# dwave-examples/image-generation

Measured on AMD Instinct MI355X. Metric: DVAE+GRBM train-step images/s (MNIST) at 1/2/4/8 MI355X; loss parity vs CPU, higher is better.
Workload: dtype f32

## Files before the change

### image-generation_amd/csrc/common.h

```cpp
#pragma once
#include <hip/hip_runtime.h>
#include <atomic>
#include <stdint.h>
#include <stdio.h>
#include <stdarg.h>
#include "../../include/dvg.h"

namespace dvg {

void set_error(const char* fmt, ...);

#define DVG_CHECK_HIP(expr)                                                            \
  do {                                                                                 \
    hipError_t _e = (expr);                                                            \
    if (_e != hipSuccess) {                                                            \
      dvg::set_error("%s failed: %s (%s:%d)", #expr, hipGetErrorString(_e), __FILE__,  \
                     __LINE__);                                                        \
      return DVG_E_HIP;                                                                \
    }                                                                                  \
  } while (0)

#define DVG_REQUIRE(cond, ...)            \
  do {                                    \
    if (!(cond)) {                        \
      dvg::set_error(__VA_ARGS__);        \
      return DVG_E_INVALID;               \
    }                                     \
  } while (0)

#define DVG_TRY(expr)          \
  do {                         \
    int _rc = (expr);          \
    if (_rc != DVG_OK) return _rc; \
  } while (0)

enum KernelId : int {
  K_GIBBS = 0,
  K_GRBM_ENERGY,
  K_GRBM_SUFFSTATS,
  K_GUMBEL_FWD,
  K_GUMBEL_BWD,
  K_MMD_PREP,
  K_MMD_DISTSUM,
  K_MMD_MAIN,
  K_MMD_PM1,
  K_MMD_FINAL,
  K_IGEMM_128x64,
  K_IGEMM_64x64,
  K_IGEMM_128x32,
  K_IGEMM_32x64,
  K_IGEMM_128x128,
  K_WGRAD_2x2,
  K_WGRAD_2x1,
  K_WGRAD_1x2,
  K_WGRAD_1x1,
  K_WGRAD_FOLD,
  K_WGRAD_REDUCE,
  K_WEIGHT_PACK,
  K_BN_FINALIZE,
  K_ENC_CONV0_FWD,
  K_ENC_CONV0_WGRAD,
  K_ENC_BN_POOL_FWD,
  K_ENC_BN_POOL_BWD_REDUCE,
  K_ENC_BN_POOL_BWD_APPLY,
  K_ENC_PROJ_FWD,
  K_ENC_PROJ_BWD,
  K_DEC_BN_ACT_FWD,
  K_DEC_BN_ACT_BWD_REDUCE,
  K_DEC_BN_ACT_BWD_APPLY,
  K_DEC_CONV3_FWD,
  K_DEC_CONV3_BWD,
  K_DEC_FINAL_FWD,
  K_DEC_FINAL_BWD,
  K_MSE,
  K_ADAM,
  K_MISC,
  K_IGEMM_WSPACE,
  K_IGEMM_WINO,
  K_WGRAD_WINO,
  K_IGEMM_WINO4,
  K_WGRAD_WINO4,
  K_COUNT
};

enum Opt : int {
  OPT_IGEMM_DMA = 0, OPT_IGEMM_POSMAJOR, OPT_IGEMM_THR128, OPT_WGRAD_DMA, OPT_DEC_FOLD, OPT_DEC_D22, OPT_DEC_LC0, OPT_MMD_W128,
  OPT_MMD_D256, OPT_GIBBS_GENERIC, OPT_SIDE_STREAM, OPT_ENC_WINO, OPT_DEC_WINO, OPT_ENC_L0_FUSED, OPT_DEC_TAIL_FUSED,
  OPT_WINO_DYNAMIC, OPT_ENC_WINO4, OPT_ENC_WINO4_MASK, OPT_ENC_DGRAD_CUS, OPT_ENC_WGRAD_CUS, OPT_DEC_WINO4_MASK, OPT_WGRAD_REDUCE_TILED, OPT_ENC_BN_REDUCE_POOLED, OPT_COUNT
};
int64_t opt(Opt id);

bool side_enabled();
void side_stream_warm();
int* dyn_tile_counters();
hipStream_t side_stream(hipStream_t fallback);
int stream_order_after(hipStream_t waiter, hipStream_t producer);
int prep_arm(const void* ws, uint64_t sig, hipStream_t producer);
int prep_join(const void* ws, uint64_t sig, hipStream_t waiter, bool* armed, bool* matched);
int stream_mark(hipStream_t producer, hipEvent_t* mark);
int stream_wait_mark(hipStream_t waiter, hipEvent_t mark);

bool prof_on(int id);
void prof_begin(int id, hipStream_t s);
void prof_end(int id, hipStream_t s, double work, float share);

struct ProfScope {
  int id; hipStream_t s; bool on; double work; float share;
  ProfScope(int id_, hipStream_t s_, double work_ = 0.0, float share_ = 1.0f) : id(id_), s(s_), on(prof_on(id_)), work(work_), share(share_) {
    if (on) prof_begin(id, s);
  }
  ~ProfScope() { if (on) prof_end(id, s, work, share); }
};

#define DVG_LAUNCH(id, kernel, grid, block, shmem, stream, ...) \
  DVG_LAUNCH_WORK(id, 0.0, kernel, grid, block, shmem, stream, __VA_ARGS__)

#define DVG_LAUNCH_WORK(id, work, kernel, grid, block, shmem, stream, ...) \
  DVG_LAUNCH_WORK_SHARE(id, work, 1.0f, kernel, grid, block, shmem, stream, __VA_ARGS__)

#define DVG_LAUNCH_WORK_SHARE(id, work, share, kernel, grid, block, shmem, stream, ...) \
  do {                                                                                  \
    dvg::ProfScope _ps((id), (stream), (work), (share));                                \
    hipLaunchKernelGGL(kernel, grid, block, shmem, stream, __VA_ARGS__);                \
    hipError_t _le = hipGetLastError();                                                 \
    if (_le != hipSuccess) {                                                            \
      dvg::set_error("launch of %s failed: %s (%s:%d)", #kernel, hipGetErrorString(_le), \
                     __FILE__, __LINE__);                                               \
      return DVG_E_HIP;                                                                 \
    }                                                                                   \
  } while (0)

static inline int raise_dynamic_lds(std::atomic<uint64_t>& done, const void* kern, int bytes) {
  int dev = 0;
  DVG_CHECK_HIP(hipGetDevice(&dev));
  const uint64_t bit = 1ull << (dev & 63);
  if (!(done.load(std::memory_order_acquire) & bit)) {
    DVG_CHECK_HIP(hipFuncSetAttribute(kern, hipFuncAttributeMaxDynamicSharedMemorySize, bytes));
    done.fetch_or(bit, std::memory_order_release);
  }
  return DVG_OK;
}

static inline int64_t ceil_div(int64_t a, int64_t b) { return (a + b - 1) / b; }
static inline size_t align_up(size_t a, size_t b) { return (a + b - 1) / b * b; }

}
```

### image-generation_amd/csrc/mmd.hip

```cpp
#include <cstdlib>
#include <type_traits>

#include "common.h"

namespace dvg {

typedef float f32x16 __attribute__((ext_vector_type(16)));
typedef float f32x4 __attribute__((ext_vector_type(4)));
typedef int i32x4 __attribute__((ext_vector_type(4)));
typedef int i32x16 __attribute__((ext_vector_type(16)));

struct MmdArgs {
  const float* x; const float* y;
  int64_t nx, ny;
  int d;
  const float* sq;
  const float* coef;
  int n_kernels, squared, reduce_mean, biased;
  int pow2;
  double* loss_part;
  int vgx = 0, vgy = 0, vgz = 0;
  float* grad_part;
  int S;
  double* dist_part;
  const int8_t* zi8;
  const int* not_pm1;
  int pm1_ok;
  int gate_main;
  const uint16_t* zt;
  int64_t ztb_y;
  const uint4* tab;
};

constexpr int MMD_BI = 32;
constexpr int MMD_BJ = 128;
constexpr int MMD_PITCH = 33;

__device__ __forceinline__ int crow(int r, int hh) { return (r & 3) + 8 * (r >> 2) + 4 * hh; }

__device__ __forceinline__ f32x16 gram_tile(const float* __restrict__ src_i, int64_t cnt_i, int64_t base_i,
                                            const float* __restrict__ src_j, int64_t cnt_j, int64_t base_j, int d,
                                            float* Zs, float* Xs) {
  const int tid = threadIdx.x, lane = tid & 63, wave = tid >> 6;
  const int hh = lane >> 5, c = lane & 31;
  f32x16 acc = {0};
  const int nchunk = d / 32;
  f32x4 zreg[4], xreg;
  float zmask[4], xmask;
  auto load_chunk = [&](int ch) {
#pragma unroll
    for (int q = 0; q < 4; ++q) {
      const int idx = tid + 256 * q;
      const int row = idx >> 3, c4 = idx & 7;
      const int64_t gr = base_j + row;
      const bool okz = gr < cnt_j;
      zreg[q] = *reinterpret_cast<const f32x4*>(src_j + (okz ? gr * d + ch * 32 + c4 * 4 : 0));
      zmask[q] = okz ? 1.0f : 0.0f;
    }
    const int row = tid >> 3, c4 = tid & 7;
    const int64_t gr = base_i + row;
    const bool okx = gr < cnt_i;
    xreg = *reinterpret_cast<const f32x4*>(src_i + (okx ? gr * d + ch * 32 + c4 * 4 : 0));
    xmask = okx ? 1.0f : 0.0f;
  };
  load_chunk(0);
  for (int ch = 0; ch < nchunk; ++ch) {
    __syncthreads();
#pragma unroll
    for (int q = 0; q < 4; ++q) {
      const int idx = tid + 256 * q;
      const int row = idx >> 3, c4 = idx & 7;
      float* p = Zs + row * MMD_PITCH + c4 * 4;
      p[0] = zreg[q].x * zmask[q]; p[1] = zreg[q].y * zmask[q]; p[2] = zreg[q].z * zmask[q]; p[3] = zreg[q].w * zmask[q];
    }
    {
      const int row = tid >> 3, c4 = tid & 7;
      float* p = Xs + row * MMD_PITCH + c4 * 4;
      p[0] = xreg.x * xmask; p[1] = xreg.y * xmask; p[2] = xreg.z * xmask; p[3] = xreg.w * xmask;
    }
    __syncthreads();
    if (ch + 1 < nchunk) load_chunk(ch + 1);
    const float* za = Zs + (wave * 32 + c) * MMD_PITCH + hh;
    const float* xb = Xs + c * MMD_PITCH + hh;
#pragma unroll
    for (int s = 0; s < 16; ++s) acc = __builtin_amdgcn_mfma_f32_32x32x2f32(za[2 * s], xb[2 * s], acc, 0, 0, 0);
  }
  return acc;
}

constexpr int MMD_I8_PANEL = 512;

template <int ROWS>
struct I8Stage {
  i32x4 v[ROWS / 32][4];
  __device__ __forceinline__ void load(const int8_t* __restrict__ src, int d, int64_t base, int64_t cnt, int n16) {
    const int tr = threadIdx.x >> 3, tc = threadIdx.x & 7;
#pragma unroll
    for (int q = 0; q < 4; ++q) {
      if (q * 8 < n16) {
        const int c16 = q * 8 + tc < n16 ? q * 8 + tc : n16 - 1;
#pragma unroll
        for (int p = 0; p < ROWS / 32; ++p) {
          int64_t gr = base + tr + 32 * p;
          gr = gr < cnt ? gr : cnt - 1;
          v[p][q] = *reinterpret_cast<const i32x4*>(src + gr * d + c16 * 16);
        }
      }
    }
  }
  __device__ __forceinline__ void store(int8_t* dst, int pitch, int n16) const {
    const int tr = threadIdx.x >> 3, tc = threadIdx.x & 7;
#pragma unroll
    for (int q = 0; q < 4; ++q) {
      if (q * 8 < n16) {
        const int c16 = q * 8 + tc < n16 ? q * 8 + tc : n16 - 1;
#pragma unroll
        for (int p = 0; p < ROWS / 32; ++p)
          *reinterpret_cast<i32x4*>(dst + (tr + 32 * p) * pitch + c16 * 16) = v[p][q];
      }
    }
  }
};

__device__ __forceinline__ f32x16 gram_tile_i8(const int8_t* __restrict__ zi8, int64_t goff_i, int64_t cnt_i,
                                               int64_t base_i, int64_t goff_j, int64_t cnt_j, int64_t base_j, int d,
                                               int8_t* Zs8, int8_t* Xs8) {
  const int tid = threadIdx.x, lane = tid & 63, wave = tid >> 6;
  const int hh = lane >> 5, c = lane & 31;
  const int pw = d < MMD_I8_PANEL ? d : MMD_I8_PANEL;
  const int pitch = pw + 16;
  i32x16 acc = {0};
  for (int c0 = 0; c0 < d; c0 += MMD_I8_PANEL) {
    const int cw = d - c0 < MMD_I8_PANEL ? d - c0 : MMD_I8_PANEL;
    const int n16 = cw >> 4;
    I8Stage<MMD_BJ> zst;
    I8Stage<MMD_BI> xst;
    zst.load(zi8 + goff_j * d + c0, d, base_j, cnt_j, n16);
    xst.load(zi8 + goff_i * d + c0, d, base_i, cnt_i, n16);
    __syncthreads();
    zst.store(Zs8, pitch, n16);
    xst.store(Xs8, pitch, n16);
    __syncthreads();
    const int8_t* za = Zs8 + (wave * 32 + c) * pitch + hh * 16;
    const int8_t* xb = Xs8 + c * pitch + hh * 16;
    for (int s = 0; s < (cw >> 5); ++s)
      acc = __builtin_amdgcn_mfma_i32_32x32x32_i8(*reinterpret_cast<const i32x4*>(za + s * 32),
                                                  *reinterpret_cast<const i32x4*>(xb + s * 32), acc, 0, 0, 0);
  }
  f32x16 out;
#pragma unroll
  for (int r = 0; r < 16; ++r) out[r] = (float)acc[r];
  return out;
}

__device__ __forceinline__ void mmd_pair_terms(float D, const float (&ck)[8], int nk, bool pow2, float& ks, float& kp) {
  ks = 0.f; kp = 0.f;
  if (pow2) {
    float e = expf(ck[nk - 1] * D);
#pragma unroll
    for (int k = 7; k >= 0; --k) {
      if (k < nk) {
        ks += e;
        kp = fmaf(ck[k], e, kp);
        e *= e;
      }
    }
  } else {
#pragma unroll
    for (int k = 0; k < 8; ++k) {
      if (k < nk) {
        const float e = expf(ck[k] * D);
        ks += e;
        kp = fmaf(ck[k], e, kp);
      }
    }
  }
}

__device__ __forceinline__ double block_sum(double v, double* red) {
  const int tid = threadIdx.x;
  red[tid] = v;
  __syncthreads();
  for (int s = 128; s > 0; s >>= 1) {
    if (tid < s) red[tid] += red[tid + s];
    __syncthreads();
  }
  const double r = red[0];
  __syncthreads();
  return r;
}

__global__ __launch_bounds__(256) void mmd_prep_kernel(const float* __restrict__ x, int64_t nx,
                                                       const float* __restrict__ y, int64_t ny, int d,
                                                       float* __restrict__ sq, int8_t* __restrict__ zi8,
                                                       int* __restrict__ not_pm1) {
  const int64_t row = (int64_t)blockIdx.x * 4 + (threadIdx.x >> 6);
  const int lane = threadIdx.x & 63;
  if (row >= nx + ny) return;
  const float* p = row < nx ? x + row * d : y + (row - nx) * d;
  float acc = 0.f;
  bool bad = false;
  uint32_t* z4 = reinterpret_cast<uint32_t*>(zi8 + row * d);
  for (int k = lane; k < d / 4; k += 64) {
    const float4 v = *reinterpret_cast<const float4*>(p + 4 * k);
    acc = fmaf(v.x, v.x, acc); acc = fmaf(v.y, v.y, acc); acc = fmaf(v.z, v.z, acc); acc = fmaf(v.w, v.w, acc);
    bad |= !(v.x == 1.0f || v.x == -1.0f) | !(v.y == 1.0f || v.y == -1.0f) | !(v.z == 1.0f || v.z == -1.0f) | !(v.w == 1.0f || v.w == -1.0f);
    z4[k] = (v.x > 0.f ? 0x01u : 0xffu) | (v.y > 0.f ? 0x0100u : 0xff00u) | (v.z > 0.f ? 0x010000u : 0xff0000u) |
            (v.w > 0.f ? 0x01000000u : 0xff000000u);
  }
  if (__any(bad) && lane == 0) atomicOr(not_pm1, 1);
#pragma unroll
  for (int off = 32; off > 0; off >>= 1) acc += __shfl_down(acc, off, 64);
  if (lane == 0) sq[row] = acc;
}

template <int NS>
__device__ __forceinline__ void mmd_distsum_spin128(const MmdArgs& a, unsigned char* dsm) {
  double* red = reinterpret_cast<double*>(dsm);
  float* Dtab = reinterpret_cast<float*>(dsm + 2048);
  const int d = a.d, pw = d < MMD_I8_PANEL ? d : MMD_I8_PANEL, zp = pw + 16;
  int8_t* Zs8 = reinterpret_cast<int8_t*>(dsm + 2048 + ((d + 1) * 4 + 15) / 16 * 16);
  for (int h = threadIdx.x; h <= d; h += 256) {
    const float d2 = (float)(4 * h);
    Dtab[h] = a.squared ? d2 : sqrtf(d2);
  }
  const int64_t tx = (a.nx + MMD_BJ - 1) / MMD_BJ, ty = (a.ny + MMD_BJ - 1) / MMD_BJ, T = tx + ty;
  const int lane = threadIdx.x & 63, wave = threadIdx.x >> 6, hh = lane >> 5, c = lane & 31;
  const int nsteps = d >> 5;
  double total = 0.0;
  for (int seg = 0; seg < 2; ++seg) {
    const int64_t g = seg == 0 ? (int64_t)blockIdx.x : T - 1 - (int64_t)blockIdx.x;
    if (g >= T || (seg == 1 && g <= (int64_t)blockIdx.x)) break;
    const bool rows_x = g < tx;
    const int64_t cnt_i = rows_x ? a.nx : a.ny, base_i = (rows_x ? g : g - tx) * 128, goff_i = rows_x ? 0 : a.nx;
    const int64_t gi = base_i + wave * 32 + c;
    const bool vi = gi < cnt_i;
    i32x4 xb[NS];
    {
      const int8_t* xrow = a.zi8 + (goff_i + (vi ? gi : cnt_i - 1)) * d + hh * 16;
#pragma unroll
      for (int s = 0; s < NS; ++s) xb[s] = s < nsteps ? *reinterpret_cast<const i32x4*>(xrow + s * 32) : (i32x4){0, 0, 0, 0};
    }
    I8Stage<MMD_BJ> zst;
    auto tile_src = [&](int64_t t, const int8_t*& src, int64_t& base_j, int64_t& cnt_j) {
      const bool cx = t < tx;
      src = a.zi8 + (cx ? 0 : a.nx) * d;
      base_j = (cx ? t : t - tx) * MMD_BJ;
      cnt_j = cx ? a.nx : a.ny;
    };
    int64_t t = g + blockIdx.y;
    if (t < T) {
      const int8_t* src; int64_t bj, cj;
      tile_src(t, src, bj, cj);
      zst.load(src, d, bj, cj, pw >> 4);
    }
    for (; t < T; t += gridDim.y) {
      const int8_t* src; int64_t base_j, cnt_j;
      tile_src(t, src, base_j, cnt_j);
      i32x16 acc[4];
#pragma unroll
      for (int jt = 0; jt < 4; ++jt) acc[jt] = (i32x16){0};
      for (int c0 = 0; c0 < d; c0 += MMD_I8_PANEL) {
        const int cw = d - c0 < MMD_I8_PANEL ? d - c0 : MMD_I8_PANEL;
        if (c0 > 0) zst.load(src + c0, d, base_j, cnt_j, cw >> 4);
        __syncthreads();
        zst.store(Zs8, zp, cw >> 4);
        __syncthreads();
        const int s0 = c0 >> 5;
#pragma unroll
        for (int s = 0; s < NS; ++s) {
          if (s >= s0 && s < s0 + (cw >> 5)) {
#pragma unroll
            for (int jt = 0; jt < 4; ++jt) {
              const i32x4 za = *reinterpret_cast<const i32x4*>(Zs8 + (jt * 32 + c) * zp + (s - s0) * 32 + hh * 16);
              acc[jt] = __builtin_amdgcn_mfma_i32_32x32x32_i8(za, xb[s], acc[jt], 0, 0, 0);
            }
          }
        }
      }
      {
        const int64_t tn = t + gridDim.y;
        if (tn < T) {
          const int8_t* nsrc; int64_t nbj, ncj;
          tile_src(tn, nsrc, nbj, ncj);
          zst.load(nsrc, d, nbj, ncj, pw >> 4);
        }
      }
      const float wgt = t == g ? 1.0f : 2.0f;
      float part = 0.f;
      if (base_i + 128 <= cnt_i && base_j + MMD_BJ <= cnt_j) {
#pragma unroll
        for (int jt = 0; jt < 4; ++jt)
#pragma unroll
          for (int r = 0; r < 16; ++r) part += Dtab[(d - acc[jt][r]) >> 1];
      } else {
#pragma unroll
        for (int jt = 0; jt < 4; ++jt)
#pragma unroll
          for (int r = 0; r < 16; ++r) {
            const int64_t gj = base_j + jt * 32 + crow(r, hh);
            const float D = Dtab[(d - acc[jt][r]) >> 1];
            part += (vi && gj < cnt_j) ? D : 0.f;
          }
      }
      total += (double)(part * wgt);
    }
  }
  const double sum = block_sum(total, red);
  if (threadIdx.x == 0) a.dist_part[(size_t)blockIdx.y * gridDim.x + blockIdx.x] = sum;
}

__device__ __forceinline__ void mmd_distsum_generic(const MmdArgs& a, unsigned char* dsm, bool I8) {
  double* red = reinterpret_cast<double*>(dsm);
  float* Zs = reinterpret_cast<float*>(dsm + 2048);
  float* Xs = Zs + MMD_BJ * MMD_PITCH;
  int8_t* Zs8 = reinterpret_cast<int8_t*>(dsm + 2048);
  int8_t* Xs8 = Zs8 + MMD_BJ * ((a.d < MMD_I8_PANEL ? a.d : MMD_I8_PANEL) + 16);
  const int64_t rbx = (a.nx + MMD_BI - 1) / MMD_BI, rby = (a.ny + MMD_BI - 1) / MMD_BI;
  const int64_t tx = (a.nx + MMD_BJ - 1) / MMD_BJ, ty = (a.ny + MMD_BJ - 1) / MMD_BJ;
  const int lane = threadIdx.x & 63, wave = threadIdx.x >> 6, hh = lane >> 5, c = lane & 31;
  double total = 0.0;
  for (int64_t rb = blockIdx.x; rb < rbx + rby; rb += gridDim.x) {
    const bool rows_x = rb < rbx;
    const float* src_i = rows_x ? a.x : a.y;
    const int64_t cnt_i = rows_x ? a.nx : a.ny, base_i = (rows_x ? rb : rb - rbx) * MMD_BI;
    const float* sq_i = rows_x ? a.sq : a.sq + a.nx;
    const int64_t gi = base_i + c;
    const float sqi = gi < cnt_i ? sq_i[gi] : 0.f;
    for (int64_t t = blockIdx.y; t < tx + ty; t += gridDim.y) {
      const bool cols_x = t < tx;
      const float* src_j = cols_x ? a.x : a.y;
      const int64_t cnt_j = cols_x ? a.nx : a.ny, base_j = (cols_x ? t : t - tx) * MMD_BJ;
      const float* sq_j = cols_x ? a.sq : a.sq + a.nx;
      f32x16 Tt;
      if (I8) Tt = gram_tile_i8(a.zi8, rows_x ? 0 : a.nx, cnt_i, base_i, cols_x ? 0 : a.nx, cnt_j, base_j, a.d, Zs8, Xs8);
      else Tt = gram_tile(src_i, cnt_i, base_i, src_j, cnt_j, base_j, a.d, Zs, Xs);
      float part = 0.f;
#pragma unroll
      for (int r = 0; r < 16; ++r) {
        const int64_t gj = base_j + wave * 32 + crow(r, hh);
        if (gi < cnt_i && gj < cnt_j) {
          const float d2 = fmaxf(sqi + sq_j[gj] - 2.0f * Tt[r], 0.f);
          part += a.squared ? d2 : sqrtf(d2);
        }
      }
      total += (double)part;
      __syncthreads();
    }
  }
  const double s = block_sum(total, red);
  if (threadIdx.x == 0) a.dist_part[(size_t)blockIdx.y * gridDim.x + blockIdx.x] = s;
}

template <int NST>
__device__ __forceinline__ void mmd_distsum_spin256(const MmdArgs& a, unsigned char* dsm) {
  constexpr int D = 32 * NST, CH = 32 * D, NPW = NST / 4;
  typedef __attribute__((address_space(3))) void lds_void;
  double* red = reinterpret_cast<double*>(dsm);
  float* Dtab = reinterpret_cast<float*>(dsm + 2048);
  unsigned char* zbuf = dsm + 2048 + ((D + 1) * 4 + 1023) / 1024 * 1024;
  for (int h = threadIdx.x; h <= D; h += 256) {
    const float d2 = (float)(4 * h);
    Dtab[h] = a.squared ? d2 : sqrtf(d2);
  }
  const int N = (int)(a.nx + a.ny);
  const int T = (N + 255) >> 8, TC = (N + 31) >> 5;
  int bx = (int)blockIdx.x, by = (int)blockIdx.y;
  if ((gridDim.y & 7) == 0) {
    const int lin = (int)(blockIdx.x + blockIdx.y * gridDim.x), per = (int)gridDim.y >> 3;
    const int idx = lin >> 3;
    by = (lin & 7) + 8 * (idx % per);
    bx = idx / per;
  }
  const int lane = threadIdx.x & 63, hh = lane >> 5, c = lane & 31;
  const int wave = __builtin_amdgcn_readfirstlane(threadIdx.x >> 6);
  const __amdgpu_buffer_rsrc_t rsrc = __builtin_amdgcn_make_buffer_rsrc(const_cast<int8_t*>(a.zi8), 0, N * D, 0x00020000);
  int poff[NPW];
#pragma unroll
  for (int q = 0; q < NPW; ++q) {
    const int byte = (wave * NPW + q) * 1024 + lane * 16;
    const int r = byte / D, sl = (byte % D) >> 4;
    const int f = (D % 256 == 0) ? (r & 15) : ((r >> 1) & 7);
    poff[q] = r * D + ((sl ^ f) << 4);
  }
  auto issue = [&](int t, int buf) {
    unsigned char* dst = zbuf + buf * CH + wave * NPW * 1024;
#pragma unroll
    for (int q = 0; q < NPW; ++q)
      __builtin_amdgcn_raw_ptr_buffer_load_lds(rsrc, (lds_void*)(dst + q * 1024), 16, poff[q], t * CH, 0, 0);
  };
  const int fc = (D % 256 == 0) ? (c & 15) : ((c >> 1) & 7);
  constexpr int tb2 = 2048 + 2 * D;
  typedef __attribute__((address_space(3))) const float lds_cfloat;
  typedef __attribute__((address_space(3))) unsigned char lds_byte;
  typedef __attribute__((address_space(3))) const i32x4 lds_ci32x4;
  if ((uint32_t)(uintptr_t)(lds_byte*)dsm != 0u) __builtin_trap();
  uint32_t zaddr[8];
#pragma unroll
  for (int j = 0; j < 8; ++j)
    zaddr[j] = (uint32_t)(2048 + ((D + 1) * 4 + 1023) / 1024 * 1024) + (uint32_t)(c * D + ((((hh ^ fc) ^ (2 * j)) & 15) << 4));
  double total = 0.0;
  __syncthreads();
  const int S = (int)gridDim.y, NB = (int)gridDim.x;
  auto seglen = [&](int g) { const int r = TC - g * 8 - by; return r > 0 ? (r + S - 1) / S : 0; };
  auto walk_g = [&](int q) { return (q & 1) ? T - 1 - (q >> 1) : (q >> 1); };
  int walk_total = 0;
  for (int q = 0; q < T; ++q) walk_total += seglen(walk_g(q));
  const int per = (walk_total + NB - 1) / NB;
  const int lo = bx * per, hi = lo + per < walk_total ? lo + per : walk_total;
  int base = 0;
  for (int q = 0; q < T && base < hi; ++q) {
    const int g = walk_g(q), len = seglen(g);
    const int k0 = lo > base ? lo - base : 0, k1 = hi - base < len ? hi - base : len;
    base += len;
    if (k1 <= k0) continue;
    i32x4 xb[2][NST];
    bool vi[2];
#pragma unroll
    for (int rs = 0; rs < 2; ++rs) {
      const int gi = g * 256 + wave * 64 + rs * 32 + c;
      vi[rs] = gi < N;
      const int8_t* xrow = a.zi8 + (int64_t)(vi[rs] ? gi : N - 1) * D + hh * 16;
#pragma unroll
      for (int s = 0; s < NST; ++s) {
        const i32x4 w = *reinterpret_cast<const i32x4*>(xrow + s * 32);
#pragma unroll
        for (int u = 0; u < 4; ++u) xb[rs][s][u] = (int)((((uint32_t)w[u] << 1) & 0xFEFEFEFEu) ^ 0xFCFCFCFCu);
      }
    }
    const int t0 = g * 8 + by + S * k0, t_end = g * 8 + by + S * k1, t_own_end = g * 8 + 8;
    float part[2] = {0.f, 0.f};
    double segsum[2] = {0.0, 0.0};
    auto lookups = [&](const i32x16& g0, const i32x16& g1, int t, bool masked) {
      float p0 = 0.f, p1 = 0.f;
#pragma unroll
      for (int r = 0; r < 16; ++r) {
        const float d0 = *reinterpret_cast<lds_cfloat*>((uintptr_t)(uint32_t)(g0[r] + tb2));
        const float d1 = *reinterpret_cast<lds_cfloat*>((uintptr_t)(uint32_t)(g1[r] + tb2));
        const bool vj = !masked || t * 32 + crow(r, hh) < N;
        p0 += vj ? d0 : 0.f;
        p1 += vj ? d1 : 0.f;
      }
      const float wgt = t < t_own_end ? 1.0f : 2.0f;
      part[0] = fmaf(p0, wgt, part[0]);
      part[1] = fmaf(p1, wgt, part[1]);
    };
    issue(t0, 0);
    int tp = -1, since_flush = 0;
    constexpr int PF = NST >= 16 ? 4 : (NST >= 8 ? 2 : 1);
    auto chunk = [&](int t, auto bufc, const i32x16 (&prev)[2], i32x16 (&cur)[2]) {
      constexpr int buf = decltype(bufc)::value;
      asm volatile("s_waitcnt vmcnt(0)" ::: "memory");
      __syncthreads();
      if (t + S < t_end) issue(t + S, buf ^ 1);
      auto zread = [&](int st) -> i32x4 {
        return *reinterpret_cast<lds_ci32x4*>((uintptr_t)(zaddr[st & 7] + (uint32_t)(buf * CH + (st >> 3) * 256)));
      };
      auto rb = [](int st) { return (16 * st) / NST; };
      i32x4 zr[NST];
      float lk0[16], lk1[16], p0 = 0.f, p1 = 0.f;
#pragma unroll
      for (int s = 0; s < PF; ++s) zr[s] = zread(s);
      __builtin_amdgcn_sched_barrier(0);
#pragma unroll
      for (int s = 0; s < NST; ++s) {
#pragma unroll
        for (int r = rb(s); r < rb(s + 1); ++r) {
          lk0[r] = *reinterpret_cast<lds_cfloat*>((uintptr_t)(uint32_t)(prev[0][r] + tb2));
          lk1[r] = *reinterpret_cast<lds_cfloat*>((uintptr_t)(uint32_t)(prev[1][r] + tb2));
        }
        if (s + PF < NST) zr[s + PF] = zread(s + PF);
        __builtin_amdgcn_sched_barrier(0);
        cur[0] = __builtin_amdgcn_mfma_i32_32x32x32_i8(zr[s], xb[0][s], s == 0 ? (i32x16){0} : cur[0], 0, 0, 0);
        cur[1] = __builtin_amdgcn_mfma_i32_32x32x32_i8(zr[s], xb[1][s], s == 0 ? (i32x16){0} : cur[1], 0, 0, 0);
        if (s >= PF) {
#pragma unroll
          for (int r = rb(s - PF); r < rb(s - PF + 1); ++r) { p0 += lk0[r]; p1 += lk1[r]; }
        }
        __builtin_amdgcn_sched_barrier(0);
      }
#pragma unroll
      for (int r = rb(NST - PF); r < 16; ++r) { p0 += lk0[r]; p1 += lk1[r]; }
      const float wgt = tp < 0 ? 0.0f : (tp < t_own_end ? 1.0f : 2.0f);
      part[0] = fmaf(p0, wgt, part[0]);
      part[1] = fmaf(p1, wgt, part[1]);
      tp = t;
      if (++since_flush == 16) {
        segsum[0] += (double)part[0]; segsum[1] += (double)part[1];
        part[0] = 0.f; part[1] = 0.f;
        since_flush = 0;
      }
    };
    i32x16 accp[2], accq[2];
    accp[0] = (i32x16){0}; accp[1] = (i32x16){0};
    bool last_in_q = false;
    for (int t = t0; t < t_end; t += 2 * S) {
      chunk(t, std::integral_constant<int, 0>{}, accp, accq);
      last_in_q = true;
      if (t + S >= t_end) break;
      chunk(t + S, std::integral_constant<int, 1>{}, accq, accp);
      last_in_q = false;
    }
    if (last_in_q) { accp[0] = accq[0]; accp[1] = accq[1]; }
    if (tp >= 0) lookups(accp[0], accp[1], tp, tp * 32 + 32 > N);
    segsum[0] += (double)part[0]; segsum[1] += (double)part[1];
    total += (vi[0] ? segsum[0] : 0.0) + (vi[1] ? segsum[1] : 0.0);
    __syncthreads();
  }
  const double sum = block_sum(total, red);
  if (threadIdx.x == 0) a.dist_part[(size_t)by * gridDim.x + bx] = sum;
}

template <int NST>
__global__ __launch_bounds__(256, 2) void mmd_distsum_spin256_kernel(MmdArgs a) {
  extern __shared__ __align__(16) unsigned char dsm[];
  if (*a.not_pm1 == 0) mmd_distsum_spin256<NST>(a, dsm);
  else mmd_distsum_generic(a, dsm, false);
}

template <int NS>
__global__ __launch_bounds__(256, NS <= 16 ? 2 : 1) void mmd_distsum_spin_kernel(MmdArgs a) {
  extern __shared__ __align__(16) unsigned char dsm[];
  if (*a.not_pm1 == 0) mmd_distsum_spin128<NS>(a, dsm);
  else mmd_distsum_generic(a, dsm, false);
}

__global__ __launch_bounds__(256) void mmd_distsum_kernel(MmdArgs a) {
  extern __shared__ __align__(16) unsigned char dsm[];
  mmd_distsum_generic(a, dsm, *a.not_pm1 == 0);
}

__device__ __forceinline__ double mmd_wave_sum(double v) {
#pragma unroll
  for (int off = 32; off > 0; off >>= 1) v += __shfl_xor(v, off, 64);
  return v;
}

template <int NFB>
__device__ __forceinline__ void mmd_main_body(const MmdArgs& a, float* smem, int vbx, int vby, int vbz, int vgx, int vgy) {
  float* Zs = smem;
  float* Xs = Zs + MMD_BJ * MMD_PITCH;
  float* Gs = Xs + MMD_BI * MMD_PITCH;
  float* rs_s = Gs + NFB * 32 * MMD_PITCH;
  double* red = reinterpret_cast<double*>(rs_s + 4 * 32 + 2);

  const int64_t rbx = (a.nx + MMD_BI - 1) / MMD_BI;
  const int64_t rb = vbx;
  const bool rows_x = rb < rbx;
  const int zslice = vbz;
  if (!rows_x && zslice > 0) return;
  const float* src_i = rows_x ? a.x : a.y;
  const int64_t cnt_i = rows_x ? a.nx : a.ny, base_i = (rows_x ? rb : rb - rbx) * MMD_BI;
  const float* sq_i = rows_x ? a.sq : a.sq + a.nx;
  const int64_t tx = (a.nx + MMD_BJ - 1) / MMD_BJ, ty = (a.ny + MMD_BJ - 1) / MMD_BJ;
  const int tid = threadIdx.x, lane = tid & 63, wave = tid >> 6, hh = lane >> 5, c = lane & 31;
  const int64_t gi = base_i + c;
  const bool vi = gi < cnt_i;
  const float sqi = vi ? sq_i[gi] : 0.f;
  const int f0 = zslice * NFB * 32;

  float ck[8];
#pragma unroll
  for (int k = 0; k < 8; ++k) ck[k] = a.coef[k];
  const float kscale = a.reduce_mean ? 1.0f / (float)a.n_kernels : 1.0f;
  const int nk = a.n_kernels;
  const double dnx = (double)a.nx, dny = (double)a.ny;
  const float a_xx = (float)(2.0 / (a.biased ? dnx * dnx : dnx * (dnx - 1.0)));
  const float a_xy = (float)(-2.0 / (dnx * dny));

  f32x16 G[NFB];
#pragma unroll
  for (int fb = 0; fb < NFB; ++fb) G[fb] = (f32x16){0};
  float rowsum = 0.f;
  double l_xx = 0.0, l_xy = 0.0, l_yy = 0.0;

  const int64_t t_begin = rows_x ? 0 : tx;
  for (int64_t t = t_begin + vby; t < tx + ty; t += vgy) {
    const bool cols_x = t < tx;
    const float* src_j = cols_x ? a.x : a.y;
    const int64_t cnt_j = cols_x ? a.nx : a.ny, base_j = (cols_x ? t : t - tx) * MMD_BJ;
    const float* sq_j = cols_x ? a.sq : a.sq + a.nx;
    f32x16 T = gram_tile(src_i, cnt_i, base_i, src_j, cnt_j, base_j, a.d, Zs, Xs);

    const bool same = (rows_x == cols_x);
    const float aw = cols_x ? a_xx : a_xy;
    float w[16];
    float lsum = 0.f;
#pragma unroll
    for (int r = 0; r < 16; ++r) {
      const int64_t gj = base_j + wave * 32 + crow(r, hh);
      float wv = 0.f;
      if (vi && gj < cnt_j) {
        const bool diag = same && (gi == gj);
        const float d2 = diag ? 0.f : fmaxf(sqi + sq_j[gj] - 2.0f * T[r], 0.f);
        const float D = a.squared ? d2 : sqrtf(d2);
        float ks, kp;
        mmd_pair_terms(D, ck, nk, a.pow2, ks, kp);
        if (a.biased || !diag) lsum += ks * kscale;
        if (rows_x) {
          const float dD = a.squared ? 2.0f : (D > 0.f ? 1.0f / D : 0.f);
          wv = diag ? 0.f : aw * kscale * kp * dD;
        }
      }
      w[r] = wv;
      rowsum += wv;
    }
    if (rows_x) { if (cols_x) l_xx += (double)lsum; else l_xy += (double)lsum; }
    else l_yy += (double)lsum;

    if (rows_x && a.grad_part) {
      const int f = f0 + c;
#pragma unroll
      for (int r = 0; r < 16; ++r) {
        const int64_t gj = base_j + wave * 32 + crow(r, hh);
        const bool vj = gj < cnt_j;
#pragma unroll
        for (int fb = 0; fb < NFB; ++fb) {
          const int ff = f + fb * 32;
          const bool oka = vj && ff < a.d;
          const float av = src_j[oka ? gj * a.d + ff : 0] * (oka ? 1.0f : 0.0f);
          G[fb] = __builtin_amdgcn_mfma_f32_32x32x2f32(av, w[r], G[fb], 0, 0, 0);
        }
      }
    }
  }

  const double sxx = block_sum(l_xx, red), sxy = block_sum(l_xy, red), syy = block_sum(l_yy, red);
  if (tid == 0 && zslice == 0) {
    double* lp = a.loss_part + ((size_t)vby * vgx + vbx) * 3;
    lp[0] = sxx; lp[1] = sxy; lp[2] = syy;
  }
  if (!rows_x || !a.grad_part) return;

  rowsum += __shfl_xor(rowsum, 32, 64);
  if (hh == 0) rs_s[wave * 32 + c] = rowsum;
  for (int wv = 0; wv < 4; ++wv) {
    if (wave == wv) {
#pragma unroll
      for (int fb = 0; fb < NFB; ++fb)
#pragma unroll
        for (int r = 0; r < 16; ++r) {
          float* p = Gs + (fb * 32 + crow(r, hh)) * MMD_PITCH + c;
          *p = (wv == 0) ? G[fb][r] : *p + G[fb][r];
        }
    }
    __syncthreads();
  }
  float* out = a.grad_part + (size_t)vby * a.nx * a.d;
  for (int e = tid; e < MMD_BI * NFB * 32; e += 256) {
    const int i = e / (NFB * 32), fl = e % (NFB * 32);
    const int64_t gr = base_i + i;
    const int ff = f0 + fl;
    if (gr < a.nx && ff < a.d) {
      const float rsum = (rs_s[i] + rs_s[32 + i]) + (rs_s[64 + i] + rs_s[96 + i]);
      out[gr * a.d + ff] = a.x[gr * a.d + ff] * rsum - Gs[fl * MMD_PITCH + i];
    }
  }
}



typedef __bf16 bf16x8 __attribute__((ext_vector_type(8)));

__device__ __forceinline__ void mmd_table_entry(const MmdArgs& a, const float (&ck)[8], int h, uint4* __restrict__ tab) {
  const float kscale = a.reduce_mean ? 1.0f / (float)a.n_kernels : 1.0f;
  const double dnx = (double)a.nx, dny = (double)a.ny;
  const float a_xx = (float)(2.0 / (a.biased ? dnx * dnx : dnx * (dnx - 1.0)));
  const float a_xy = (float)(-2.0 / (dnx * dny));
  const float d2 = 4.0f * (float)h;
  const float D = a.squared ? d2 : sqrtf(d2);
  float ks, kp;
  mmd_pair_terms(D, ck, a.n_kernels, a.pow2, ks, kp);
  const float dD = a.squared ? 2.0f : (D > 0.f ? 1.0f / D : 0.f);
  for (int which = 0; which < 2; ++which) {
    const float aw = which == 0 ? a_xx : a_xy;
    const float w = aw * kscale * kp * dD;
    const uint32_t wb = __float_as_uint(w);
    const uint32_t hi = wb & 0xffff0000u;
    const float r1 = w - __uint_as_float(hi);
    const uint32_t mid = __float_as_uint(r1) & 0xffff0000u;
    const float r2 = r1 - __uint_as_float(mid);
    const uint32_t lo = __float_as_uint(r2) & 0xffff0000u;
    uint4 e;
    e.x = __float_as_uint(ks * kscale);
    e.y = wb;
    e.z = hi | (mid >> 16);
    e.w = lo >> 16;
    tab[(size_t)which * (a.d + 1) + h] = e;
  }
}

__global__ __launch_bounds__(256) void mmd_bandwidth_table_kernel(MmdArgs a, const double* __restrict__ part, int nparts,
                                                                  double n_total, float fixed_bw, float factor,
                                                                  float* __restrict__ coef, uint4* __restrict__ tab) {
  __shared__ float ck_s[8];
  if (threadIdx.x < 64) {
    double s = 0.0;
    for (int k = threadIdx.x; k < nparts; k += 64) s += part[k];
    s = mmd_wave_sum(s);
    if (threadIdx.x == 0) {
      const double bw = fixed_bw > 0.f ? (double)fixed_bw : s / (n_total * n_total - n_total);
      const float bwf = (float)bw;
      coef[8] = bwf;
      for (int k = 0; k < 8; ++k) {
        float cv = 0.f;
        if (k < a.n_kernels) cv = -1.0f / (bwf * powf(factor, (float)(k - a.n_kernels / 2)));
        coef[k] = cv;
        ck_s[k] = cv;
      }
    }
  }
  __syncthreads();
  if (!tab || *a.not_pm1 != 0) return;
  float ck[8];
#pragma unroll
  for (int k = 0; k < 8; ++k) ck[k] = ck_s[k];
  for (int h = threadIdx.x; h <= a.d; h += 256) mmd_table_entry(a, ck, h, tab);
}

__global__ __launch_bounds__(256) void mmd_prep_fused_kernel(MmdArgs a, float* __restrict__ sq, int8_t* __restrict__ zi8,
                                                             int* __restrict__ not_pm1, uint16_t* __restrict__ zt,
                                                             int zero_loss_parts) {
  extern __shared__ __align__(16) unsigned char prep_smem[];
  const int tid = threadIdx.x, lane = tid & 63, wave = tid >> 6, d = a.d, pitch = d + 16;
  for (int64_t e = (int64_t)blockIdx.x * 256 + tid; e < 3 * (int64_t)zero_loss_parts; e += (int64_t)gridDim.x * 256)
    a.loss_part[e] = 0.0;
  const int64_t jb = blockIdx.x;
  const bool is_x = jb < a.ztb_y;
  const int64_t cnt = is_x ? a.nx : a.ny, row0 = (is_x ? jb : jb - a.ztb_y) * 32, goff = is_x ? 0 : a.nx;
  const float* src = is_x ? a.x : a.y;
  float acc[8];
#pragma unroll
  for (int u = 0; u < 8; ++u) acc[u] = 0.f;
  bool bad = false;
  for (int k = lane; k < d / 4; k += 64) {
    float4 v[8];
#pragma unroll
    for (int u = 0; u < 8; ++u) {
      const int64_t row = row0 + wave + 4 * u;
      v[u] = row < cnt ? *reinterpret_cast<const float4*>(src + row * d + 4 * k) : make_float4(1.f, 1.f, 1.f, 1.f);
    }
#pragma unroll
    for (int u = 0; u < 8; ++u) {
      const int64_t row = row0 + wave + 4 * u;
      const float4 w = v[u];
      acc[u] = fmaf(w.x, w.x, acc[u]); acc[u] = fmaf(w.y, w.y, acc[u]); acc[u] = fmaf(w.z, w.z, acc[u]); acc[u] = fmaf(w.w, w.w, acc[u]);
      bad |= !(w.x == 1.0f || w.x == -1.0f) | !(w.y == 1.0f || w.y == -1.0f) | !(w.z == 1.0f || w.z == -1.0f) | !(w.w == 1.0f || w.w == -1.0f);
      const uint32_t z = (w.x > 0.f ? 0x01u : 0xffu) | (w.y > 0.f ? 0x0100u : 0xff00u) | (w.z > 0.f ? 0x010000u : 0xff0000u) |
                         (w.w > 0.f ? 0x01000000u : 0xff000000u);
      *reinterpret_cast<uint32_t*>(prep_smem + (wave + 4 * u) * pitch + 4 * k) = z;
      if (row < cnt) reinterpret_cast<uint32_t*>(zi8 + (goff + row) * d)[k] = z;
    }
  }
  if (__any(bad) && lane == 0) atomicOr(not_pm1, 1);
#pragma unroll
  for (int u = 0; u < 8; ++u) {
    float t = acc[u];
#pragma unroll
    for (int off = 32; off > 0; off >>= 1) t += __shfl_down(t, off, 64);
    const int64_t row = row0 + wave + 4 * u;
    if (lane == 0 && row < cnt) sq[goff + row] = t;
  }
  __syncthreads();
  for (int f = tid; f < d; f += 256) {
    uint32_t packed[16];
#pragma unroll
    for (int q = 0; q < 16; ++q) {
      uint32_t v = 0;
#pragma unroll
      for (int half = 0; half < 2; ++half) {
        const int k = 2 * q + half, sgrp = k >> 4, hh = (k >> 3) & 1, e = k & 7;
        const int r = 16 * sgrp + 8 * (e >> 2) + 4 * hh + (e & 3);
        const uint32_t b = row0 + r < cnt ? ((int8_t)prep_smem[r * pitch + f] > 0 ? 0x3f80u : 0xbf80u) : 0u;
        v |= b << (16 * half);
      }
      packed[q] = v;
    }
    uint4* dst = reinterpret_cast<uint4*>(zt + (jb * d + f) * 32);
#pragma unroll
    for (int q = 0; q < 4; ++q) dst[q] = make_uint4(packed[4 * q], packed[4 * q + 1], packed[4 * q + 2], packed[4 * q + 3]);
  }
}

template <int NFB>
__device__ __forceinline__ void mmd_pm1_body(const MmdArgs& a, unsigned char* pm1_smem) {
  const int d = a.d;
  const int pw = d < MMD_I8_PANEL ? d : MMD_I8_PANEL;
  const int zp = pw + 16, xp = d + 16;
  uint4* tab_s = reinterpret_cast<uint4*>(pm1_smem);
  float* rs_s = reinterpret_cast<float*>(tab_s + 2 * (d + 1));
  double* red = reinterpret_cast<double*>(rs_s + 128);
  int8_t* Xs8 = reinterpret_cast<int8_t*>(red + 256);
  int8_t* Zs8 = Xs8 + MMD_BI * xp;
  float* Gs = reinterpret_cast<float*>(Zs8);

  const int64_t rbx = (a.nx + MMD_BI - 1) / MMD_BI;
  const int64_t rb = blockIdx.x;
  const bool rows_x = rb < rbx;
  const int zslice = blockIdx.z;
  if (!rows_x && zslice > 0) return;
  const int64_t cnt_i = rows_x ? a.nx : a.ny, base_i = (rows_x ? rb : rb - rbx) * MMD_BI;
  const int64_t goff_i = rows_x ? 0 : a.nx;
  const int64_t tx = (a.nx + MMD_BJ - 1) / MMD_BJ, ty = (a.ny + MMD_BJ - 1) / MMD_BJ;
  const int tid = threadIdx.x, lane = tid & 63, wave = tid >> 6, hh = lane >> 5, c = lane & 31;
  const int64_t gi = base_i + c;
  const bool vi = gi < cnt_i;
  const int f0 = zslice * NFB * 32;
  const bool want_grad = rows_x && a.grad_part != nullptr;

  for (int e = tid; e < 2 * (d + 1); e += 256) tab_s[e] = a.tab[e];
  for (int c0 = 0; c0 < d; c0 += MMD_I8_PANEL) {
    const int cw = d - c0 < MMD_I8_PANEL ? d - c0 : MMD_I8_PANEL;
    I8Stage<MMD_BI> xst;
    xst.load(a.zi8 + goff_i * d + c0, d, base_i, cnt_i, cw >> 4);
    xst.store(Xs8 + c0, xp, cw >> 4);
  }

  f32x16 G[NFB];
#pragma unroll
  for (int fb = 0; fb < NFB; ++fb) G[fb] = (f32x16){0};
  float rowsum = 0.f;
  double l_xx = 0.0, l_xy = 0.0, l_yy = 0.0;

  const int64_t t_begin = rows_x ? 0 : tx;
  I8Stage<MMD_BJ> zst;
  {
    const int64_t t0 = t_begin + blockIdx.y;
    if (t0 < tx + ty) {
      const bool x0 = t0 < tx;
      zst.load(a.zi8 + (x0 ? 0 : a.nx) * d, d, (x0 ? t0 : t0 - tx) * MMD_BJ, x0 ? a.nx : a.ny, pw >> 4);
    }
  }
  for (int64_t t = t_begin + blockIdx.y; t < tx + ty; t += gridDim.y) {
    const bool cols_x = t < tx;
    const int64_t cnt_j = cols_x ? a.nx : a.ny, base_j = (cols_x ? t : t - tx) * MMD_BJ;
    const int64_t goff_j = cols_x ? 0 : a.nx;

    i32x16 acc = {0};
    for (int c0 = 0; c0 < d; c0 += MMD_I8_PANEL) {
      const int cw = d - c0 < MMD_I8_PANEL ? d - c0 : MMD_I8_PANEL;
      const int n16 = cw >> 4;
      if (c0 > 0) zst.load(a.zi8 + goff_j * d + c0, d, base_j, cnt_j, n16);
      __syncthreads();
      zst.store(Zs8, zp, n16);
      __syncthreads();
      const int8_t* za = Zs8 + (wave * 32 + c) * zp + hh * 16;
      const int8_t* xb = Xs8 + c * xp + c0 + hh * 16;
      for (int s = 0; s < (cw >> 5); ++s)
        acc = __builtin_amdgcn_mfma_i32_32x32x32_i8(*reinterpret_cast<const i32x4*>(za + s * 32),
                                                    *reinterpret_cast<const i32x4*>(xb + s * 32), acc, 0, 0, 0);
    }
    {
      const int64_t tn = t + gridDim.y;
      if (tn < tx + ty) {
        const bool nx_ = tn < tx;
        zst.load(a.zi8 + (nx_ ? 0 : a.nx) * d, d, (nx_ ? tn : tn - tx) * MMD_BJ, nx_ ? a.nx : a.ny, pw >> 4);
      }
    }

    const bool same = (rows_x == cols_x);
    const uint4* tb = tab_s + (cols_x ? 0 : d + 1);
    uint32_t himid[16], lo[16];
    float lsum = 0.f;
    const int nj = (int)(cnt_j - base_j < MMD_BJ ? cnt_j - base_j : MMD_BJ);
    const int64_t dd = gi - base_j;
    const int dloc = (same && !a.biased && dd >= 0 && dd < MMD_BJ) ? (int)dd : -1;
    const i32x4* tb4 = reinterpret_cast<const i32x4*>(tb);
#pragma unroll
    for (int r = 0; r < 16; ++r) {
      const int jl = wave * 32 + crow(r, hh);
      const int h = (d - acc[r]) >> 1;
      const i32x4 e = tb4[h];
      const uint32_t vm = (vi && jl < nj) ? 0xffffffffu : 0u;
      const uint32_t lm = jl != dloc ? vm : 0u;
      const uint32_t wm = rows_x ? vm : 0u;
      lsum += __uint_as_float((uint32_t)e[0] & lm);
      rowsum += __uint_as_float((uint32_t)e[1] & wm);
      himid[r] = (uint32_t)e[2] & wm;
      lo[r] = (uint32_t)e[3] & wm;
    }
    if (rows_x) { if (cols_x) l_xx += (double)lsum; else l_xy += (double)lsum; }
    else l_yy += (double)lsum;

    if (want_grad) {
      i32x4 Bw[2][3];
#pragma unroll
      for (int s = 0; s < 2; ++s)
#pragma unroll
        for (int q = 0; q < 4; ++q) {
          const int r = 8 * s + 2 * q;
          Bw[s][0][q] = (int)__builtin_amdgcn_perm(himid[r + 1], himid[r], 0x07060302u);
          Bw[s][1][q] = (int)__builtin_amdgcn_perm(himid[r + 1], himid[r], 0x05040100u);
          Bw[s][2][q] = (int)__builtin_amdgcn_perm(lo[r + 1], lo[r], 0x05040100u);
        }
      const int64_t jb = (cols_x ? 0 : a.ztb_y) + base_j / 32 + wave;
      const uint16_t* zrow = a.zt + (jb * d + f0 + c) * 32 + 8 * hh;
      constexpr int PF = NFB < 4 ? NFB : 4;
      i32x4 av[2][PF][2];
      auto load_group = [&](int g, i32x4 (&dst)[PF][2]) {
#pragma unroll
        for (int u = 0; u < PF; ++u)
#pragma unroll
          for (int s = 0; s < 2; ++s) {
            const int fb = g * PF + u;
            dst[u][s] = *reinterpret_cast<const i32x4*>(zrow + (size_t)fb * 32 * 32 + 16 * s);
          }
      };
      load_group(0, av[0]);
#pragma unroll
      for (int g = 0; g < NFB / PF; ++g) {
        if (g + 1 < NFB / PF) load_group(g + 1, av[(g + 1) & 1]);
        __builtin_amdgcn_sched_barrier(0);
#pragma unroll
        for (int u = 0; u < PF; ++u)
#pragma unroll
          for (int s = 0; s < 2; ++s)
#pragma unroll
            for (int term = 0; term < 3; ++term)
              G[g * PF + u] = __builtin_amdgcn_mfma_f32_32x32x16_bf16(__builtin_bit_cast(bf16x8, av[g & 1][u][s]),
                                                                      __builtin_bit_cast(bf16x8, Bw[s][term]),
                                                                      G[g * PF + u], 0, 0, 0);
        __builtin_amdgcn_sched_barrier(0);
      }
    }
  }

  const double sxx = block_sum(l_xx, red), sxy = block_sum(l_xy, red), syy = block_sum(l_yy, red);
  if (tid == 0 && zslice == 0) {
    double* lp = a.loss_part + ((size_t)blockIdx.y * gridDim.x + blockIdx.x) * 3;
    lp[0] = sxx; lp[1] = sxy; lp[2] = syy;
  }
  if (!want_grad) return;

  rowsum += __shfl_xor(rowsum, 32, 64);
  if (hh == 0) rs_s[wave * 32 + c] = rowsum;
  __syncthreads();
  for (int wv = 0; wv < 4; ++wv) {
    if (wave == wv) {
#pragma unroll
      for (int fb = 0; fb < NFB; ++fb)
#pragma unroll
        for (int r = 0; r < 16; ++r) {
          float* p = Gs + (fb * 32 + crow(r, hh)) * MMD_PITCH + c;
          *p = (wv == 0) ? G[fb][r] : *p + G[fb][r];
        }
    }
    __syncthreads();
  }
  float* out = a.grad_part + (size_t)blockIdx.y * a.nx * d;
  for (int e = tid; e < MMD_BI * NFB * 32; e += 256) {
    const int i = e / (NFB * 32), fl = e % (NFB * 32);
    const int64_t gr = base_i + i;
    const int ff = f0 + fl;
    if (gr < a.nx && ff < d) {
      const float rsum = (rs_s[i] + rs_s[32 + i]) + (rs_s[64 + i] + rs_s[96 + i]);
      out[gr * d + ff] = a.x[gr * d + ff] * rsum - Gs[fl * MMD_PITCH + i];
    }
  }
}

template <int NFBW>
__device__ __forceinline__ void mmd_pm1_fq_body(const MmdArgs& a, unsigned char* pm1_smem) {
  constexpr int NFB = 4 * NFBW;
  const int d = a.d;
  const int pw = d < MMD_I8_PANEL ? d : MMD_I8_PANEL;
  const int zp = pw + 16, xp = d + 16;
  uint4* tab_s = reinterpret_cast<uint4*>(pm1_smem);
  float* rs_s = reinterpret_cast<float*>(tab_s + 2 * (d + 1));
  double* red = reinterpret_cast<double*>(rs_s + 128);
  int8_t* Xs8 = reinterpret_cast<int8_t*>(red + 256);
  int8_t* Zs8 = Xs8 + MMD_BI * xp;
  float* Gs = reinterpret_cast<float*>(Zs8);
  i32x4* wx = reinterpret_cast<i32x4*>(Zs8 + (((size_t)MMD_BJ * zp > sizeof(float) * NFB * 32 * MMD_PITCH ? (size_t)MMD_BJ * zp : sizeof(float) * NFB * 32 * MMD_PITCH) + 15) / 16 * 16);

  const int64_t rbx = (a.nx + MMD_BI - 1) / MMD_BI;
  const int64_t rb = blockIdx.x;
  const bool rows_x = rb < rbx;
  if (blockIdx.z > 0) return;
  constexpr int zslice = 0;
  const int64_t cnt_i = rows_x ? a.nx : a.ny, base_i = (rows_x ? rb : rb - rbx) * MMD_BI;
  const int64_t goff_i = rows_x ? 0 : a.nx;
  const int64_t tx = (a.nx + MMD_BJ - 1) / MMD_BJ, ty = (a.ny + MMD_BJ - 1) / MMD_BJ;
  const int tid = threadIdx.x, lane = tid & 63, wave = tid >> 6, hh = lane >> 5, c = lane & 31;
  const int64_t gi = base_i + c;
  const bool vi = gi < cnt_i;
  const int f0 = (tid >> 6) * NFBW * 32;
  const bool want_grad = rows_x && a.grad_part != nullptr;

  for (int e = tid; e < 2 * (d + 1); e += 256) tab_s[e] = a.tab[e];
  for (int c0 = 0; c0 < d; c0 += MMD_I8_PANEL) {
    const int cw = d - c0 < MMD_I8_PANEL ? d - c0 : MMD_I8_PANEL;
    I8Stage<MMD_BI> xst;
    xst.load(a.zi8 + goff_i * d + c0, d, base_i, cnt_i, cw >> 4);
    xst.store(Xs8 + c0, xp, cw >> 4);
  }

  f32x16 G[NFBW];
#pragma unroll
  for (int fb = 0; fb < NFBW; ++fb) G[fb] = (f32x16){0};
  float rowsum = 0.f;
  double l_xx = 0.0, l_xy = 0.0, l_yy = 0.0;

  const int64_t t_begin = rows_x ? 0 : tx;
  I8Stage<MMD_BJ> zst;
  {
    const int64_t t0 = t_begin + blockIdx.y;
    if (t0 < tx + ty) {
      const bool x0 = t0 < tx;
      zst.load(a.zi8 + (x0 ? 0 : a.nx) * d, d, (x0 ? t0 : t0 - tx) * MMD_BJ, x0 ? a.nx : a.ny, pw >> 4);
    }
  }
  for (int64_t t = t_begin + blockIdx.y; t < tx + ty; t += gridDim.y) {
    const bool cols_x = t < tx;
    const int64_t cnt_j = cols_x ? a.nx : a.ny, base_j = (cols_x ? t : t - tx) * MMD_BJ;
    const int64_t goff_j = cols_x ? 0 : a.nx;

    i32x16 acc = {0};
    for (int c0 = 0; c0 < d; c0 += MMD_I8_PANEL) {
      const int cw = d - c0 < MMD_I8_PANEL ? d - c0 : MMD_I8_PANEL;
      const int n16 = cw >> 4;
      if (c0 > 0) zst.load(a.zi8 + goff_j * d + c0, d, base_j, cnt_j, n16);
      __syncthreads();
      zst.store(Zs8, zp, n16);
      __syncthreads();
      const int8_t* za = Zs8 + (wave * 32 + c) * zp + hh * 16;
      const int8_t* xb = Xs8 + c * xp + c0 + hh * 16;
      for (int s = 0; s < (cw >> 5); ++s)
        acc = __builtin_amdgcn_mfma_i32_32x32x32_i8(*reinterpret_cast<const i32x4*>(za + s * 32),
                                                    *reinterpret_cast<const i32x4*>(xb + s * 32), acc, 0, 0, 0);
    }
    {
      const int64_t tn = t + gridDim.y;
      if (tn < tx + ty) {
        const bool nx_ = tn < tx;
        zst.load(a.zi8 + (nx_ ? 0 : a.nx) * d, d, (nx_ ? tn : tn - tx) * MMD_BJ, nx_ ? a.nx : a.ny, pw >> 4);
      }
    }

    const bool same = (rows_x == cols_x);
    const uint4* tb = tab_s + (cols_x ? 0 : d + 1);
    uint32_t himid[16], lo[16];
    float lsum = 0.f;
    const int nj = (int)(cnt_j - base_j < MMD_BJ ? cnt_j - base_j : MMD_BJ);
    const int64_t dd = gi - base_j;
    const int dloc = (same && !a.biased && dd >= 0 && dd < MMD_BJ) ? (int)dd : -1;
    const i32x4* tb4 = reinterpret_cast<const i32x4*>(tb);
#pragma unroll
    for (int r = 0; r < 16; ++r) {
      const int jl = wave * 32 + crow(r, hh);
      const int h = (d - acc[r]) >> 1;
      const i32x4 e = tb4[h];
      const uint32_t vm = (vi && jl < nj) ? 0xffffffffu : 0u;
      const uint32_t lm = jl != dloc ? vm : 0u;
      const uint32_t wm = rows_x ? vm : 0u;
      lsum += __uint_as_float((uint32_t)e[0] & lm);
      rowsum += __uint_as_float((uint32_t)e[1] & wm);
      himid[r] = (uint32_t)e[2] & wm;
      lo[r] = (uint32_t)e[3] & wm;
    }
    if (rows_x) { if (cols_x) l_xx += (double)lsum; else l_xy += (double)lsum; }
    else l_yy += (double)lsum;

    if (want_grad) {
      i32x4 Bw[2][3];
#pragma unroll
      for (int s = 0; s < 2; ++s)
#pragma unroll
        for (int q = 0; q < 4; ++q) {
          const int r = 8 * s + 2 * q;
          Bw[s][0][q] = (int)__builtin_amdgcn_perm(himid[r + 1], himid[r], 0x07060302u);
          Bw[s][1][q] = (int)__builtin_amdgcn_perm(himid[r + 1], himid[r], 0x05040100u);
          Bw[s][2][q] = (int)__builtin_amdgcn_perm(lo[r + 1], lo[r], 0x05040100u);
        }
#pragma unroll
      for (int s = 0; s < 2; ++s)
#pragma unroll
        for (int term = 0; term < 3; ++term) wx[((wave * 2 + s) * 3 + term) * 64 + lane] = Bw[s][term];
      __syncthreads();
      const uint16_t* zbase = a.zt + (((cols_x ? 0 : a.ztb_y) + base_j / 32) * d + f0 + c) * 32 + 8 * hh;
      i32x4 av[2][2][NFBW];
      auto load_jb = [&](int jb, i32x4 (&dst)[2][NFBW]) {
#pragma unroll
        for (int s = 0; s < 2; ++s)
#pragma unroll
          for (int fb = 0; fb < NFBW; ++fb)
            dst[s][fb] = *reinterpret_cast<const i32x4*>(zbase + ((size_t)jb * d + fb * 32) * 32 + 16 * s);
      };
      load_jb(0, av[0]);
#pragma unroll
      for (int jb = 0; jb < 4; ++jb) {
        if (jb + 1 < 4) load_jb(jb + 1, av[(jb + 1) & 1]);
        __builtin_amdgcn_sched_barrier(0);
#pragma unroll
        for (int s = 0; s < 2; ++s)
#pragma unroll
          for (int term = 0; term < 3; ++term) {
            const i32x4 bw = wx[((jb * 2 + s) * 3 + term) * 64 + lane];
#pragma unroll
            for (int fb = 0; fb < NFBW; ++fb)
              G[fb] = __builtin_amdgcn_mfma_f32_32x32x16_bf16(__builtin_bit_cast(bf16x8, av[jb & 1][s][fb]),
                                                              __builtin_bit_cast(bf16x8, bw), G[fb], 0, 0, 0);
          }
        __builtin_amdgcn_sched_barrier(0);
      }
    }
  }

  const double sxx = block_sum(l_xx, red), sxy = block_sum(l_xy, red), syy = block_sum(l_yy, red);
  if (tid == 0 && zslice == 0) {
    double* lp = a.loss_part + ((size_t)blockIdx.y * gridDim.x + blockIdx.x) * 3;
    lp[0] = sxx; lp[1] = sxy; lp[2] = syy;
  }
  if (!want_grad) return;

  rowsum += __shfl_xor(rowsum, 32, 64);
  if (hh == 0) rs_s[wave * 32 + c] = rowsum;
  __syncthreads();
#pragma unroll
  for (int fb = 0; fb < NFBW; ++fb)
#pragma unroll
    for (int r = 0; r < 16; ++r) Gs[(wave * NFBW * 32 + fb * 32 + crow(r, hh)) * MMD_PITCH + c] = G[fb][r];
  __syncthreads();
  float* out = a.grad_part + (size_t)blockIdx.y * a.nx * d;
  for (int e = tid; e < MMD_BI * NFB * 32; e += 256) {
    const int i = e / (NFB * 32), fl = e % (NFB * 32);
    const int64_t gr = base_i + i;
    const int ff = fl;
    if (gr < a.nx && ff < d) {
      const float rsum = (rs_s[i] + rs_s[32 + i]) + (rs_s[64 + i] + rs_s[96 + i]);
      out[gr * d + ff] = a.x[gr * d + ff] * rsum - Gs[fl * MMD_PITCH + i];
    }
  }
}

template <int NST, int NFT, bool ONE = false>
struct W128 {
  static constexpr int D = 32 * NST;
  static constexpr int TABN = D + 3;
  static constexpr int TAB_BYTES = ((ONE ? 1 : 2) * TABN * 8 + 1023) / 1024 * 1024;
  static constexpr int RED_BYTES = 2048;
  static constexpr int Z8_BYTES = 32 * D;
  static constexpr int ZT_BYTES = 64 * 32 * NFT;
  static constexpr int NSTG = 3;
  static constexpr int OFF_RED = TAB_BYTES, OFF_Z8 = OFF_RED + RED_BYTES, OFF_ZT = OFF_Z8 + NSTG * Z8_BYTES;
  static constexpr int LDS_BYTES = OFF_ZT + NSTG * ZT_BYTES;
  static_assert(LDS_BYTES <= 160 * 1024, "w128: LDS image over the CU's 160 KiB");
};

__device__ __forceinline__ void dma16(const void* gsrc, unsigned char* lds_wave_base) {
  __builtin_amdgcn_global_load_lds((const void __attribute__((address_space(1)))*)gsrc,
                                   (void __attribute__((address_space(3)))*)lds_wave_base, 16, 0, 0);
}

template <int NST, int NFT, bool ONE = false>
__device__ __forceinline__ void mmd_pm1_w128_body(const MmdArgs& a, unsigned char* smem) {
  using L = W128<NST, NFT, ONE>;
  constexpr int D = L::D;
  typedef __attribute__((address_space(3))) void lds_void;
  typedef __attribute__((address_space(3))) unsigned char lds_byte;
  typedef int i32x2 __attribute__((ext_vector_type(2)));
  double* red = reinterpret_cast<double*>(smem + L::OFF_RED);
  unsigned char* z8buf = smem + L::OFF_Z8;
  unsigned char* ztbuf = smem + L::OFF_ZT;

  const int tid = threadIdx.x, lane = tid & 63, wave = __builtin_amdgcn_readfirstlane(tid >> 6), hh = lane >> 5, c = lane & 31;
  const int64_t rbx = (a.nx + 127) / 128;
  int rb_i = blockIdx.x, sp_i = blockIdx.y, zc_i = blockIdx.z;
  if (gridDim.z > 1) {
    const int GX = gridDim.x, S = gridDim.y, nbx = (int)rbx, nby = GX - nbx;
    int lin = blockIdx.x + GX * (blockIdx.y + S * blockIdx.z);
    const int ngrad = nbx * S * gridDim.z;
    const bool gx = lin < ngrad;
    lin = gx ? lin : lin - ngrad;
    const int nb = gx ? nbx : nby;
    rb_i = (gx ? 0 : nbx) + lin % nb; sp_i = (lin / nb) % S; zc_i = lin / (nb * S);
  }
  const int64_t rb = rb_i;
  const bool rows_x = rb < rbx;
  const int sp = sp_i;
  if (!rows_x && sp > 0) return;
  const int64_t cnt_i = rows_x ? a.nx : a.ny, base_i = (rows_x ? rb : rb - rbx) * 128, goff_i = rows_x ? 0 : a.nx;
  const int64_t gi = base_i + wave * 32 + c;
  const bool vi = gi < cnt_i;
  const int f0 = zc_i * 32 * NFT;
  const bool want_grad = rows_x && a.grad_part != nullptr;
  const int zc = zc_i, nzc = gridDim.z;
  const int64_t ncx = (a.nx + 31) / 32, ncy = (a.ny + 31) / 32;
  int64_t t0, t1;
  if (rows_x) {
    const int64_t nc = ncx + ncy, per = (nc + gridDim.y - 1) / gridDim.y;
    t0 = sp * per; t1 = t0 + per < nc ? t0 + per : nc;
  } else {
    t0 = ncx; t1 = ncx + ncy;
  }
  if (!want_grad && nzc > 1) {
    const int64_t per = (t1 - t0 + nzc - 1) / nzc, u0 = t0 + zc * per;
    t1 = u0 + per < t1 ? u0 + per : t1;
    t0 = u0;
  }
  const int T = t1 > t0 ? (int)(t1 - t0) : 0;
  const int ncx_i = (int)ncx, nx_i = (int)a.nx, ny_i = (int)a.ny, gi_i = (int)gi, base_i_i = (int)base_i;

  constexpr int TABN = L::TABN;
  const int one_which = (rows_x && t0 < (int64_t)((a.nx + 31) / 32)) ? 0 : 1;
  for (int e = tid; e < (ONE ? 1 : 2) * TABN; e += 256) {
    const int which = ONE ? one_which : e / TABN, h = ONE ? e : e - which * TABN;
    uint4 v = make_uint4(0u, 0u, 0u, 0u);
    if (h <= D) v = a.tab[which * (D + 1) + h];
    else if (h == D + 2) { v = a.tab[which * (D + 1)]; v.x = 0u; }
    const float w = __uint_as_float(v.y);
    auto rn_bf16 = [](float f) { const uint32_t u = __float_as_uint(f); return (u + 0x7fffu + ((u >> 16) & 1u)) & 0xffff0000u; };
    const uint32_t hi = rn_bf16(w);
    const uint32_t lo = rn_bf16(w - __uint_as_float(hi));
    reinterpret_cast<uint2*>(smem)[e] = make_uint2(v.x, hi | (lo >> 16));
  }
  i32x4 xb[NST];
  {
    const int8_t* xrow = a.zi8 + (goff_i + (vi ? gi : cnt_i - 1)) * D + hh * 16;
#pragma unroll
    for (int s = 0; s < NST; ++s) xb[s] = *reinterpret_cast<const i32x4*>(xrow + s * 32);
  }

  constexpr int NZ8 = NST / 4, NZT = NFT / 2;
  int z8off[NZ8], ztoff0;
#pragma unroll
  for (int q = 0; q < NZ8; ++q) {
    const int byte = (wave * NZ8 + q) * 1024 + lane * 16;
    const int r = byte / D, sl = (byte % D) >> 4;
    const int fz = (D % 256 == 0) ? (r & 15) : ((r >> 1) & 7);
    z8off[q] = r * D + ((sl ^ fz) << 4);
  }
  {
    const int f = wave * NZT * 16 + (lane >> 2), sl = lane & 3;
    ztoff0 = f * 64 + ((sl ^ ((f >> 2) & 3)) << 4);
  }
  const __amdgpu_buffer_rsrc_t rsrc8 = __builtin_amdgcn_make_buffer_rsrc(const_cast<int8_t*>(a.zi8), 0, (int)((a.nx + a.ny) * D), 0x00020000);
  const __amdgpu_buffer_rsrc_t rsrct = __builtin_amdgcn_make_buffer_rsrc(
      const_cast<uint16_t*>(a.zt), 0, (int)((a.ztb_y + (a.ny + 127) / 128 * 4) * (int64_t)D * 64), 0x00020000);
  const uint32_t lds0 = (uint32_t)__builtin_amdgcn_readfirstlane((int)(uint32_t)(uintptr_t)(lds_byte*)smem);
  const int tl_i = (int)t1 - 1;
  auto z8_soff = [&](int t) -> int {
    t = t < tl_i ? t : tl_i;
    const bool cx = t < ncx_i;
    return ((cx ? 0 : nx_i) + (cx ? t : t - ncx_i) * 32) * D;
  };
  auto zt_soff = [&](int t) -> int {
    t = t < tl_i ? t : tl_i;
    const bool cx = t < ncx_i;
    return (((cx ? 0 : (int)a.ztb_y) + (cx ? t : t - ncx_i)) * D + f0) * 64;
  };
  auto issue_z8 = [&](int t, int stg) {
    const int so = __builtin_amdgcn_readfirstlane(z8_soff(t));
    const uint32_t dst = lds0 + (uint32_t)(L::OFF_Z8 + stg * L::Z8_BYTES + wave * NZ8 * 1024);
#pragma unroll
    for (int q = 0; q < NZ8; ++q)
      __builtin_amdgcn_raw_ptr_buffer_load_lds(rsrc8, (lds_void*)(uintptr_t)(dst + q * 1024), 16, z8off[q], so, 0, 0);
  };
  auto issue_zt = [&](int t, int stg) {
    const int so = __builtin_amdgcn_readfirstlane(zt_soff(t));
    const uint32_t dst = lds0 + (uint32_t)(L::OFF_ZT + stg * L::ZT_BYTES + wave * NZT * 1024);
#pragma unroll
    for (int q = 0; q < NZT; ++q)
      __builtin_amdgcn_raw_ptr_buffer_load_lds(rsrct, (lds_void*)(uintptr_t)(dst + q * 1024), 16, ztoff0, so + q * 1024, 0, 0);
  };

  const int fz_c = (D % 256 == 0) ? (c & 15) : ((c >> 1) & 7);
  const int sw_c = (c >> 2) & 3;
  const int aoff0 = c * 64 + ((hh ^ sw_c) << 4), aoff1 = c * 64 + (((2 + hh) ^ sw_c) << 4);
  constexpr int ZSW = (D % 256 == 0) ? 16 : 8;
  constexpr int NZB = ZSW / 2 < NST ? ZSW / 2 : NST;
  int zlow[NZB];
#pragma unroll
  for (int m = 0; m < NZB; ++m) zlow[m] = c * D + (((2 * m + hh) ^ fz_c) << 4);

  auto gram = [&](int stg) -> i32x16 {
    const unsigned char* z = z8buf + stg * L::Z8_BYTES;
    i32x16 acc = {0};
#pragma unroll
    for (int s = 0; s < NST; ++s) {
      const i32x4 za = *reinterpret_cast<const i32x4*>(z + zlow[s % NZB] + (s / NZB) * (ZSW * 16));
      acc = __builtin_amdgcn_mfma_i32_32x32x32_i8(za, xb[s], acc, 0, 0, 0);
    }
    return acc;
  };

  f32x16 G[NFT];
#pragma unroll
  for (int ft = 0; ft < NFT; ++ft) G[ft] = (f32x16){0};

  struct ChunkMeta { bool cols_x, fix; int nj, djrow; };
  const bool diag_kind = !a.biased;
  auto chunk_meta = [&](int t, bool exists) -> ChunkMeta {
    ChunkMeta m;
    m.cols_x = t < ncx_i;
    const int jrow0 = (m.cols_x ? t : t - ncx_i) * 32, cnt_j = m.cols_x ? nx_i : ny_i;
    const int left = cnt_j - jrow0;
    m.nj = exists ? (left < 32 ? left : 32) : 0;
    const bool diag_here = exists && diag_kind && rows_x == m.cols_x && jrow0 + 32 > base_i_i && jrow0 < base_i_i + 128;
    m.djrow = diag_here ? jrow0 : -(1 << 30);
    m.fix = m.nj < 32 || diag_here;
    return m;
  };
  auto fixup = [&](i32x16& S, const ChunkMeta& m) {
    int hho = hh;
    asm volatile("" : "+v"(hho));
    const int dloc = gi_i - m.djrow;
#pragma unroll
    for (int r = 0; r < 16; ++r) {
      const int jl = crow(r, hho);
      int v = S[r];
      v = jl == dloc ? -(D + 4) : v;
      v = jl < m.nj ? v : -(D + 2);
      S[r] = v;
    }
  };

  float lsum = 0.f, rs_hi = 0.f, rs_lo = 0.f;
  uint32_t hm_prev = 0;
  constexpr int NTERM = 2;
  auto look_issue = [&](const i32x16& S, int r, const unsigned char* tb) -> i32x2 {
    return *reinterpret_cast<const i32x2*>(tb + __mul24(S[r], -4));
  };
  auto look_use = [&](const i32x2& e, int r, i32x4 (&Bn)[2][NTERM]) {
    lsum += __int_as_float(e[0]);
    const uint32_t hm = (uint32_t)e[1];
    rs_hi += __uint_as_float(hm & 0xffff0000u);
    rs_lo += __uint_as_float(hm << 16);
    asm volatile("" ::"v"(lsum), "v"(rs_hi), "v"(rs_lo));
    if (r & 1) {
      const int s2 = r >> 3, q = (r & 7) >> 1;
      Bn[s2][0][q] = (int)__builtin_amdgcn_perm(hm, hm_prev, 0x07060302u);
      Bn[s2][1][q] = (int)__builtin_amdgcn_perm(hm, hm_prev, 0x05040100u);
      asm volatile("" ::"v"(Bn[s2][0][q]), "v"(Bn[s2][1][q]));
    } else {
      hm_prev = hm;
    }
  };
  auto table_base = [&](bool cols_x) -> const unsigned char* { return smem + ((ONE || cols_x) ? 0 : TABN * 8) + 4 * D; };
  double l_cx = 0.0, l_cy = 0.0;
  double rowsum_d = 0.0;
  auto flush_lsum = [&](bool cols_x) {
    const double dl = vi ? (double)lsum : 0.0;
    l_cx += cols_x ? dl : 0.0;
    l_cy += cols_x ? 0.0 : dl;
    lsum = 0.f;
    rowsum_d += (double)rs_hi + (double)rs_lo;
    rs_hi = 0.f; rs_lo = 0.f;
  };

  i32x4 Bw[2][NTERM];
  if (T > 0 && want_grad) {
    issue_z8((int)t0, 0);
    issue_z8((int)t0 + 1, 1);
    issue_z8((int)t0 + 2, 2);
    issue_zt((int)t0, 0);
    issue_zt((int)t0 + 1, 1);
    asm volatile("s_waitcnt vmcnt(0)" ::: "memory");
    __builtin_amdgcn_s_barrier();
    {
      const ChunkMeta m = chunk_meta((int)t0, true);
      i32x16 S = gram(0);
      if (m.fix) fixup(S, m);
      const unsigned char* tb = table_base(m.cols_x);
#pragma unroll
      for (int r = 0; r < 16; ++r) look_use(look_issue(S, r, tb), r, Bw);
      flush_lsum(m.cols_x);
    }
    i32x16 Sa = gram(1), Sb = {0};
    if constexpr (NST / NFT > 1) asm volatile("" : "+v"(Sa), "+v"(Sb));
    __builtin_amdgcn_s_barrier();
    issue_z8((int)t0 + 3, 0);
    asm volatile("s_waitcnt vmcnt(0)" ::: "memory");
    if constexpr (NST / NFT == 1) asm volatile("" : "+v"(Sa), "+v"(Sb));

    auto rb = [](int ft) { return ft >= NFT - 1 ? 16 : (16 * ft + NFT - 2) / (NFT - 1); };
    constexpr int RMAX = (16 + NFT - 2) / (NFT - 1);
    constexpr int GPT = NST / NFT;
    struct Carry {
      int z8so, ztso;
      uint32_t z8dst, ztdst;
      bool fix, cols_x;
      int nj, djrow;
      bool prev_cols_x;
    };
    auto carry_for = [&](int k, int stg) -> Carry {
      Carry cy;
      const int t = (int)t0 + k;
      const int s1 = stg == 2 ? 0 : stg + 1, s2 = stg == 0 ? 2 : stg - 1;
      cy.z8so = __builtin_amdgcn_readfirstlane(z8_soff(t + 4));
      cy.ztso = __builtin_amdgcn_readfirstlane(zt_soff(t + 2));
      cy.z8dst = lds0 + (uint32_t)(L::OFF_Z8 + s1 * L::Z8_BYTES + wave * NZ8 * 1024);
      cy.ztdst = lds0 + (uint32_t)(L::OFF_ZT + s2 * L::ZT_BYTES + wave * NZT * 1024);
      const bool more = k + 1 < T;
      const ChunkMeta m = chunk_meta(more ? t + 1 : t, more);
      cy.fix = m.fix; cy.cols_x = m.cols_x; cy.nj = m.nj; cy.djrow = m.djrow;
      cy.prev_cols_x = t < ncx_i;
      return cy;
    };
    struct Addr { const unsigned char* a0; const unsigned char* a1; const unsigned char* z[NZB]; };
    auto addr_for = [&](int stg_zt, int stg_z8) -> Addr {
      Addr ad;
      ad.a0 = ztbuf + stg_zt * L::ZT_BYTES + aoff0;
      ad.a1 = ztbuf + stg_zt * L::ZT_BYTES + aoff1;
#pragma unroll
      for (int m = 0; m < NZB; ++m) ad.z[m] = z8buf + stg_z8 * L::Z8_BYTES + zlow[m];
      return ad;
    };
    auto zread = [&](const Addr& ad, int s_) -> i32x4 {
      return *reinterpret_cast<const i32x4*>(ad.z[s_ % NZB] + (s_ / NZB) * (ZSW * 16));
    };

    int stg = 0;
    Carry cy = carry_for(0, 0);
    Addr ad = addr_for(0, 2);
    i32x4 ac[2], zc[GPT];
    ac[0] = *reinterpret_cast<const i32x4*>(ad.a0);
    ac[1] = *reinterpret_cast<const i32x4*>(ad.a1);
#pragma unroll
    for (int u = 0; u < GPT; ++u) zc[u] = zread(ad, u);
    i32x2 ent[RMAX];

    auto iteration = [&](int k, auto parity, i32x16& Scur, i32x16& Snext) {
      (void)parity;
      if constexpr (GPT == 1) {
        asm volatile("s_waitcnt vmcnt(0)" ::: "memory");
        __builtin_amdgcn_s_barrier();
      }
      asm volatile("" : "+v"(Scur));
      if (cy.fix) {
        asm volatile("" ::: "memory");
        ChunkMeta m;
        m.cols_x = cy.cols_x; m.fix = true; m.nj = cy.nj; m.djrow = cy.djrow;
        fixup(Scur, m);
      }
      const unsigned char* tb = table_base(cy.cols_x);
      const Carry cur = cy;
      const int stg_n = stg == 2 ? 0 : stg + 1;
      i32x4 Bn[2][NTERM];
      i32x4 an[2], zn[GPT];
#pragma unroll
      for (int ft = 0; ft < NFT; ++ft) {
#pragma unroll
        for (int u = 0; u < GPT; ++u) asm volatile("" ::"v"(zc[u]));
        asm volatile("" ::"v"(ac[0]), "v"(ac[1]));
        if (ft > 0) {
#pragma unroll
          for (int u = 0; u < RMAX; ++u)
            if (rb(ft - 1) + u < rb(ft)) asm volatile("" ::"v"(ent[u]));
        }
        __builtin_amdgcn_sched_barrier(0);
#pragma unroll
        for (int u = 0; u < GPT; ++u) {
          if constexpr (GPT > 1) {
            if (ft == 0 && u == 0) Snext = (i32x16){0};
            Snext = __builtin_amdgcn_mfma_i32_32x32x32_i8(zc[u], xb[ft * GPT + u], Snext, 0, 0, 0);
          } else
          if (ft == 0 && u == 0)
            asm volatile("v_mfma_i32_32x32x32_i8 %0, %1, %2, 0" : "=&v"(Snext) : "v"(zc[u]), "v"(xb[ft * GPT + u]));
          else
            asm volatile("v_mfma_i32_32x32x32_i8 %0, %1, %2, %0" : "+v"(Snext) : "v"(zc[u]), "v"(xb[ft * GPT + u]));
        }
        __builtin_amdgcn_sched_barrier(0);
        if (ft + 1 < NFT) {
          an[0] = *reinterpret_cast<const i32x4*>(ad.a0 + (ft + 1) * 2048);
          an[1] = *reinterpret_cast<const i32x4*>(ad.a1 + (ft + 1) * 2048);
#pragma unroll
          for (int u = 0; u < GPT; ++u) zn[u] = zread(ad, (ft + 1) * GPT + u);
        } else {
          if constexpr (GPT > 1) {
            asm volatile("s_waitcnt vmcnt(%0)" ::"n"(NZ8 + NZT) : "memory");
            __builtin_amdgcn_s_barrier();
            asm volatile("" ::: "memory");
          }
          const int dzt = stg == 2 ? -2 * L::ZT_BYTES : L::ZT_BYTES;
          const int dz8 = stg == 0 ? -2 * L::Z8_BYTES : L::Z8_BYTES;
          ad.a0 += dzt; ad.a1 += dzt;
#pragma unroll
          for (int m = 0; m < NZB; ++m) ad.z[m] += dz8;
          an[0] = *reinterpret_cast<const i32x4*>(ad.a0);
          an[1] = *reinterpret_cast<const i32x4*>(ad.a1);
#pragma unroll
          for (int u = 0; u < GPT; ++u) zn[u] = zread(ad, u);
        }
        i32x2 enew[RMAX];
#pragma unroll
        for (int u = 0; u < RMAX; ++u)
          if (rb(ft) + u < rb(ft + 1)) enew[u] = look_issue(Scur, rb(ft) + u, tb);
        {
          constexpr int PPT = (NZ8 + NZT + NFT / 2 - 1) / (NFT / 2);
#pragma unroll
          for (int u = 0; u < PPT; ++u) {
            const int i = ft * PPT + u;
            if (i < NZ8)
              __builtin_amdgcn_raw_ptr_buffer_load_lds(rsrc8, (lds_void*)(uintptr_t)(cur.z8dst + i * 1024), 16, z8off[i], cur.z8so, 0, 0);
            else if (i < NZ8 + NZT)
              __builtin_amdgcn_raw_ptr_buffer_load_lds(rsrct, (lds_void*)(uintptr_t)(cur.ztdst + (i - NZ8) * 1024), 16, ztoff0, cur.ztso + (i - NZ8) * 1024, 0, 0);
          }
        }
#pragma unroll
        for (int term = 0; term < NTERM; ++term) {
          G[ft] = __builtin_amdgcn_mfma_f32_32x32x16_bf16(__builtin_bit_cast(bf16x8, ac[0]),
                                                          __builtin_bit_cast(bf16x8, Bw[0][term]), G[ft], 0, 0, 0);
          G[ft] = __builtin_amdgcn_mfma_f32_32x32x16_bf16(__builtin_bit_cast(bf16x8, ac[1]),
                                                          __builtin_bit_cast(bf16x8, Bw[1][term]), G[ft], 0, 0, 0);
        }
        if (ft > 0) {
#pragma unroll
          for (int u = 0; u < RMAX; ++u)
            if (rb(ft - 1) + u < rb(ft)) look_use(ent[u], rb(ft - 1) + u, Bn);
        }
        if (ft == 0) flush_lsum(cur.prev_cols_x);
        if (ft == NFT / 2) {
          cy = carry_for(k + 1, stg_n);
        }
#pragma unroll
        for (int u = 0; u < RMAX; ++u) ent[u] = enew[u];
        ac[0] = an[0]; ac[1] = an[1];
#pragma unroll
        for (int u = 0; u < GPT; ++u) zc[u] = zn[u];
        __builtin_amdgcn_sched_group_barrier(0x100, 2, 0);
        __builtin_amdgcn_sched_group_barrier(0x020, 2, 0);
#pragma unroll
        for (int i = 0; i < 2 * NTERM; ++i) {
          __builtin_amdgcn_sched_group_barrier(0x008, 1, 0);
          if (i < 2) __builtin_amdgcn_sched_group_barrier(0x100, 1, 0);
          __builtin_amdgcn_sched_group_barrier(0x002, 4, 0);
        }
        __builtin_amdgcn_sched_barrier(0);
      }
#pragma unroll
      for (int s2 = 0; s2 < 2; ++s2)
#pragma unroll
        for (int term = 0; term < NTERM; ++term) Bw[s2][term] = Bn[s2][term];
      stg = stg_n;
    };
    for (int k = 0; k < T; k += 2) {
      iteration(k, std::integral_constant<int, 0>{}, Sa, Sb);
      iteration(k + 1, std::integral_constant<int, 1>{}, Sb, Sa);
    }
    flush_lsum(cy.prev_cols_x);
    asm volatile("s_waitcnt vmcnt(0)" ::: "memory");
  } else if (T > 0) {
    issue_z8((int)t0, 0);
    if (T > 1) issue_z8((int)t0 + 1, 1);
    asm volatile("s_waitcnt vmcnt(0)" ::: "memory");
    __builtin_amdgcn_s_barrier();
    for (int k = 0; k < T; ++k) {
      const int t = (int)t0 + k;
      if (k + 2 < T) issue_z8(t + 2, (k + 2) % 3);
      const ChunkMeta m = chunk_meta(t, true);
      i32x16 S = gram(k % 3);
      if (m.fix) fixup(S, m);
      const unsigned char* tb = table_base(m.cols_x);
#pragma unroll
      for (int r = 0; r < 16; ++r) look_use(look_issue(S, r, tb), r, Bw);
      flush_lsum(m.cols_x);
      asm volatile("s_waitcnt vmcnt(0)" ::: "memory");
      __builtin_amdgcn_s_barrier();
    }
  } else {
    __syncthreads();
  }
  double l_xx = 0.0, l_xy = 0.0, l_yy = 0.0;
  if (rows_x) { l_xx = l_cx; l_xy = l_cy; } else { l_yy = l_cy; }

  const double sxx = block_sum(l_xx, red), sxy = block_sum(l_xy, red), syy = block_sum(l_yy, red);
  if (tid == 0) {
    const bool counts = !want_grad || zc == 0;
    double* lp = a.loss_part + (((size_t)zc * gridDim.y + sp) * gridDim.x + rb) * 3;
    lp[0] = counts ? sxx : 0.0; lp[1] = counts ? sxy : 0.0; lp[2] = counts ? syy : 0.0;
  }
  if (!want_grad) return;

  rowsum_d += __shfl_xor(rowsum_d, 32, 64);
  const float rowsum = (float)rowsum_d;
  if (vi) {
    float* out = a.grad_part + (size_t)sp * a.nx * D + gi * D + f0;
    const int8_t* xs = a.zi8 + gi * D + f0;
#pragma unroll
    for (int ft = 0; ft < NFT; ++ft)
#pragma unroll
      for (int q = 0; q < 4; ++q) {
        const int f = 32 * ft + 8 * q + 4 * hh;
        const uint32_t sg = *reinterpret_cast<const uint32_t*>(xs + f);
        f32x4 o;
#pragma unroll
        for (int u = 0; u < 4; ++u) {
          const bool neg = (sg >> (8 * u + 7)) & 1u;
          o[u] = (neg ? -rowsum : rowsum) - G[ft][4 * q + u];
        }
        *reinterpret_cast<f32x4*>(out + f) = o;
      }
  }
}

template <int NST, int NFT, bool ONE = false>
__global__ __launch_bounds__(256, 1) void mmd_pair_w128_kernel(MmdArgs a) {
  extern __shared__ __align__(16) unsigned char w128_smem[];
  if (*a.not_pm1 != 0) return;
  mmd_pm1_w128_body<NST, NFT, ONE>(a, w128_smem);
}

template <int NFB>
__global__ __launch_bounds__(256, 1) void mmd_main_kernel(MmdArgs a) {
  extern __shared__ __align__(16) unsigned char main_smem[];
  if (a.gate_main) {
    if (*a.not_pm1 == 0) return;
    const int gx = a.vgx, gy = a.vgy, total = gx * gy * a.vgz;
    for (int vb = blockIdx.x; vb < total; vb += gridDim.x) {
      mmd_main_body<NFB>(a, reinterpret_cast<float*>(main_smem), vb % gx, (vb / gx) % gy, vb / (gx * gy), gx, gy);
      __syncthreads();
    }
    return;
  }
  mmd_main_body<NFB>(a, reinterpret_cast<float*>(main_smem), blockIdx.x, blockIdx.y, blockIdx.z, gridDim.x, gridDim.y);
}

template <int NFBW>
__global__ __launch_bounds__(256, 1) void mmd_pair_fq_kernel(MmdArgs a) {
  extern __shared__ __align__(16) unsigned char fq_smem[];
  if (*a.not_pm1 == 0) mmd_pm1_fq_body<NFBW>(a, fq_smem);
  else mmd_main_body<(NFBW * 4 > 8 ? 8 : NFBW * 4)>(a, reinterpret_cast<float*>(fq_smem), blockIdx.x, blockIdx.y, blockIdx.z, gridDim.x, gridDim.y);
}

template <int NFB>
__global__ __launch_bounds__(256, 1) void mmd_pair_kernel(MmdArgs a) {
  extern __shared__ __align__(16) unsigned char pair_smem[];
  if (a.pm1_ok && *a.not_pm1 == 0) mmd_pm1_body<NFB>(a, pair_smem);
  else mmd_main_body<NFB>(a, reinterpret_cast<float*>(pair_smem), blockIdx.x, blockIdx.y, blockIdx.z, gridDim.x, gridDim.y);
}

__global__ __launch_bounds__(256) void mmd_final_kernel(const double* __restrict__ loss_part, int nparts, int64_t nx,
                                                        int64_t ny, int biased, float* __restrict__ loss_out,
                                                        const float* __restrict__ grad_part, int S, int64_t numel,
                                                        float* __restrict__ grad_x) {
  if (blockIdx.x == 0 && threadIdx.x < 64) {
    double sxx = 0, sxy = 0, syy = 0;
    for (int k = threadIdx.x; k < nparts; k += 64) { sxx += loss_part[3 * k]; sxy += loss_part[3 * k + 1]; syy += loss_part[3 * k + 2]; }
    sxx = mmd_wave_sum(sxx); sxy = mmd_wave_sum(sxy); syy = mmd_wave_sum(syy);
    if (threadIdx.x == 0) {
      const double dnx = (double)nx, dny = (double)ny;
      const double xx = sxx / (biased ? dnx * dnx : dnx * (dnx - 1.0));
      const double yy = syy / (biased ? dny * dny : dny * (dny - 1.0));
      *loss_out = (float)(xx + yy - 2.0 * sxy / (dnx * dny));
    }
  }
  if (grad_x && S > 1) {
    for (int64_t e = (int64_t)blockIdx.x * 256 + threadIdx.x; e < numel; e += (int64_t)gridDim.x * 256) {
      float s = 0.f;
      for (int k = 0; k < S; ++k) s += grad_part[(size_t)k * numel + e];
      grad_x[e] = s;
    }
  }
}

struct MmdPlan {
  int nfb, zslices, S, S1;
  bool d256;
  int64_t rbx, rby, GX1;
  size_t off_sq, off_coef, off_dist, off_loss, off_grad, off_flag, off_zi8, off_zt, off_tab, total;
  int pm1_ok;
  int64_t ztb_x, ztb_y;
  int w128, S2;
  int z128;
  int64_t rb128x, rb128y;
};

static int mmd_w128_env() {
  const int64_t v = opt(OPT_MMD_W128);
  return v < 0 ? -1 : (v ? 1 : 0);
}

static int64_t mmd_target_blocks() { return 256; }
static int mmd_w128_slices(int d) { return d == 1024 ? 8 : 1; }

static MmdPlan mmd_plan(int64_t nx, int64_t ny, int d) {
  MmdPlan p;
  const int fbt = d / 32;
  p.nfb = fbt <= 2 ? 2 : (fbt <= 4 ? 4 : 8);
  p.zslices = (fbt + p.nfb - 1) / p.nfb;
  p.rbx = ceil_div(nx, MMD_BI);
  p.rby = ceil_div(ny, MMD_BI);
  const int64_t tiles = ceil_div(nx, MMD_BJ) + ceil_div(ny, MMD_BJ);
  int64_t S = ceil_div(mmd_target_blocks(), p.rbx * p.zslices);
  if (S > tiles) S = tiles;
  if (S < 1) S = 1;
  if (S > 16) S = 16;
  p.S = (int)S;
  p.pm1_ok = d <= 1024;
  p.rb128x = ceil_div(nx, 128);
  p.rb128y = ceil_div(ny, 128);
  {
    const int64_t chunks = ceil_div(nx, 32) + ceil_div(ny, 32);
    const int env = mmd_w128_env();
    auto splits_for = [&](int64_t z) {
      int64_t S = ceil_div(mmd_target_blocks(), p.rb128x * z);
      if (S > chunks / 16) S = chunks / 16;
      if (S < 1) S = 1;
      if (env == 1) { if (S > 16) S = 16; } else if (S > 4) S = 4;
      return S;
    };
    int64_t z128 = mmd_w128_slices(d);
    if (d == 1024) {
      const int64_t S4 = splits_for(4), per4 = ceil_div(chunks, S4);
      if (ceil_div(nx, 32) % per4 == 0) z128 = 4;
    }
    p.z128 = (int)z128;
    int64_t S2 = ceil_div(mmd_target_blocks(), p.rb128x * z128);
    if (S2 > chunks / 16) S2 = chunks / 16;
    if (S2 < 1) S2 = 1;
    const bool shape_ok = d % 128 == 0 && (d <= 512 || d == 1024) && (int64_t)(nx + ny) * (int64_t)d * 2 < 2147483647LL;
    p.w128 = shape_ok && (env == 1 || (env != 0 && S2 <= 4 && p.rb128x * S2 * z128 >= 128));
    if (env == 1 && shape_ok) { S2 = S2 > 16 ? 16 : S2; }
    else if (S2 > 4) S2 = 4;
    p.S2 = (int)S2;
  }
  int64_t S1;
  {
    const int64_t ov = opt(OPT_MMD_D256);
    const int env = ov < 0 ? -1 : (ov ? 1 : 0);
    const int64_t t256 = ceil_div(nx + ny, 256);
    p.d256 = p.pm1_ok && env != 0 && d % 128 == 0 && d <= 512 && (t256 >= 32 || env == 1) && (nx + ny) * (int64_t)d < 2147483647LL;
  }
  if (p.d256) {
    p.GX1 = 64;
    S1 = 8;
  } else if (p.pm1_ok) {
    p.GX1 = (tiles + 1) / 2;
    S1 = ceil_div(512, p.GX1);
    if (S1 > tiles + 1) S1 = tiles + 1;
    if (S1 > 32) S1 = 32;
  } else {
    p.GX1 = p.rbx + p.rby;
    S1 = ceil_div(1024, p.GX1);
    if (S1 > tiles) S1 = tiles;
    if (S1 > 16) S1 = 16;
  }
  if (S1 < 1) S1 = 1;
  p.S1 = (int)S1;
  size_t o = 0;
  p.off_sq = o; o = align_up(o + sizeof(float) * (size_t)(nx + ny), 256);
  p.off_coef = o; o = align_up(o + sizeof(float) * 16, 256);
  p.off_dist = o; o = align_up(o + sizeof(double) * (size_t)(p.S1 * p.GX1), 256);
  {
    size_t nparts = (size_t)(p.S * (p.rbx + p.rby));
    if (p.w128 && (size_t)(p.S2 * p.z128 * (p.rb128x + p.rb128y)) > nparts) nparts = (size_t)(p.S2 * p.z128 * (p.rb128x + p.rb128y));
    if (p.w128 && (size_t)(p.S2 * (p.rbx + p.rby)) > nparts) nparts = (size_t)(p.S2 * (p.rbx + p.rby));
    p.off_loss = o; o = align_up(o + sizeof(double) * 3 * nparts, 256);
  }
  {
    const int smax = p.w128 && p.S2 > p.S ? p.S2 : p.S;
    p.off_grad = o; o = align_up(o + (smax > 1 ? sizeof(float) * (size_t)smax * (size_t)nx * (size_t)d : 0), 256);
  }
  p.ztb_x = ceil_div(nx, MMD_BJ) * 4;
  p.ztb_y = ceil_div(ny, MMD_BJ) * 4;
  p.off_flag = o; o = align_up(o + sizeof(int), 256);
  p.off_zi8 = o; o = align_up(o + (size_t)(nx + ny) * (size_t)d, 256);
  p.off_zt = o; o = align_up(o + (p.pm1_ok ? (size_t)(p.ztb_x + p.ztb_y) * (size_t)d * 32 * sizeof(uint16_t) : 0), 256);
  p.off_tab = o; o = align_up(o + (p.pm1_ok ? 2 * (size_t)(d + 1) * sizeof(uint4) : 0), 256);
  p.total = o;
  return p;
}

template <int NFB>
static int launch_main(const MmdArgs& a, const MmdPlan& p, hipStream_t s) {
  const size_t lds = sizeof(float) * (size_t)(MMD_BJ * MMD_PITCH + MMD_BI * MMD_PITCH + NFB * 32 * MMD_PITCH + 4 * 32 + 2) +
                     sizeof(double) * 256;
  auto kern = mmd_main_kernel<NFB>;
  if (lds > 64 * 1024)
    DVG_CHECK_HIP(hipFuncSetAttribute((const void*)kern, hipFuncAttributeMaxDynamicSharedMemorySize, (int)lds));
  const double N = (double)(a.nx + a.ny);
  const double flops = 2.0 * N * N * a.d + 2.0 * (double)a.nx * N * a.d;
  if (a.gate_main) {
    MmdArgs g = a;
    g.vgx = (int)(p.rbx + p.rby); g.vgy = p.S; g.vgz = p.zslices;
    const int64_t total = (int64_t)g.vgx * g.vgy * g.vgz;
    DVG_LAUNCH_WORK(K_MMD_MAIN, flops, kern, dim3((unsigned)(total < 512 ? total : 512)), dim3(256), lds, s, g);
    return DVG_OK;
  }
  DVG_LAUNCH_WORK(K_MMD_MAIN, flops, kern, dim3((unsigned)(p.rbx + p.rby), (unsigned)p.S, (unsigned)p.zslices), dim3(256), lds, s, a);
  return DVG_OK;
}

static void mmd_pm1_flops(int64_t nx_, int64_t ny_, int d_, bool grad, int terms, int gram_passes, double* i8, double* b16) {
  const double nx = (double)nx_, ny = (double)ny_, d = (double)d_;
  *i8 = 2.0 * (gram_passes * nx * (nx + ny) + ny * ny) * d;
  *b16 = grad ? terms * 2.0 * nx * (nx + ny) * d : 0.0;
}
static double mmd_pm1_work(const MmdArgs& a, int terms, int gram_passes = 1) {
  double i8, b16;
  mmd_pm1_flops(a.nx, a.ny, a.d, a.grad_part != nullptr, terms, gram_passes, &i8, &b16);
  return 0.5 * i8 + b16;
}

template <int NFBW>
static int launch_pair_fq(const MmdArgs& a, const MmdPlan& p, hipStream_t s) {
  constexpr int NFB = 4 * NFBW, NFBM = NFB > 8 ? 8 : NFB;
  const int d = a.d, pw = d < MMD_I8_PANEL ? d : MMD_I8_PANEL;
  const size_t zbytes = (size_t)MMD_BJ * (pw + 16), gbytes = sizeof(float) * NFB * 32 * MMD_PITCH;
  const size_t zg = ((zbytes > gbytes ? zbytes : gbytes) + 15) / 16 * 16;
  const size_t lds_s = 2 * (size_t)(d + 1) * sizeof(uint4) + sizeof(float) * 128 + sizeof(double) * 256 +
                       (size_t)MMD_BI * (d + 16) + zg + sizeof(i32x4) * 24 * 64;
  const size_t lds_m = sizeof(float) * (size_t)(MMD_BJ * MMD_PITCH + MMD_BI * MMD_PITCH + NFBM * 32 * MMD_PITCH + 4 * 32 + 2) +
                       sizeof(double) * 256;
  const size_t lds = lds_s > lds_m ? lds_s : lds_m;
  auto kern = mmd_pair_fq_kernel<NFBW>;
  if (lds > 64 * 1024)
    DVG_CHECK_HIP(hipFuncSetAttribute((const void*)kern, hipFuncAttributeMaxDynamicSharedMemorySize, (int)lds));
  const int zs = (d / 32 + NFBM - 1) / NFBM;
  DVG_LAUNCH_WORK(K_MMD_PM1, mmd_pm1_work(a, 3), kern, dim3((unsigned)(p.rbx + p.rby), (unsigned)p.S, (unsigned)zs), dim3(256), lds, s, a);
  return DVG_OK;
}

template <int NST, int NFT, bool ONE = false>
static int launch_pair_w128(const MmdArgs& a, const MmdPlan& p, hipStream_t s) {
  auto kern = mmd_pair_w128_kernel<NST, NFT, ONE>;
  constexpr int lds = W128<NST, NFT, ONE>::LDS_BYTES;
  if (lds > 64 * 1024)
    DVG_CHECK_HIP(hipFuncSetAttribute((const void*)kern, hipFuncAttributeMaxDynamicSharedMemorySize, lds));
  DVG_LAUNCH_WORK(K_MMD_PM1, mmd_pm1_work(a, 2, NST / NFT), kern, dim3((unsigned)(p.rb128x + p.rb128y), (unsigned)p.S2, NST / NFT),
                  dim3(256), (size_t)lds, s, a);
  return DVG_OK;
}

template <int NFB>
static int launch_pair(const MmdArgs& a, const MmdPlan& p, hipStream_t s) {
  const int d = a.d, pw = d < MMD_I8_PANEL ? d : MMD_I8_PANEL;
  const size_t zbytes = (size_t)MMD_BJ * (pw + 16), gbytes = sizeof(float) * NFB * 32 * MMD_PITCH;
  const size_t lds_s = 2 * (size_t)(d + 1) * sizeof(uint4) + sizeof(float) * 128 + sizeof(double) * 256 +
                       (size_t)MMD_BI * (d + 16) + (zbytes > gbytes ? zbytes : gbytes);
  const size_t lds_m = sizeof(float) * (size_t)(MMD_BJ * MMD_PITCH + MMD_BI * MMD_PITCH + NFB * 32 * MMD_PITCH + 4 * 32 + 2) +
                       sizeof(double) * 256;
  const size_t lds = lds_s > lds_m ? lds_s : lds_m;
  auto kern = mmd_pair_kernel<NFB>;
  if (lds > 64 * 1024)
    DVG_CHECK_HIP(hipFuncSetAttribute((const void*)kern, hipFuncAttributeMaxDynamicSharedMemorySize, (int)lds));
  const int zs = d / (32 * NFB);
  DVG_LAUNCH_WORK(K_MMD_PM1, mmd_pm1_work(a, 3), kern, dim3((unsigned)(p.rbx + p.rby), (unsigned)p.S, (unsigned)zs), dim3(256), lds, s, a);
  return DVG_OK;
}

static constexpr bool mmd_two_slices() { return false; }

}

using namespace dvg;

extern "C" int dvg_mmd_spin_flops(int64_t nx, int64_t ny, int dim, double* int8_flops, double* bf16_flops, int* bf16_terms) {
  DVG_REQUIRE(nx >= 2 && ny >= 2 && dim >= 32 && dim % 32 == 0 && int8_flops && bf16_flops && bf16_terms, "mmd_spin_flops: bad argument");
  const MmdPlan p = mmd_plan(nx, ny, dim);
  if (!p.pm1_ok) { *int8_flops = 0.0; *bf16_flops = 0.0; *bf16_terms = 0; return DVG_OK; }
  const int passes = p.w128 ? p.z128 * ((dim > 256 && dim <= 512 && mmd_two_slices()) ? 2 : 1) : 1;
  *bf16_terms = p.w128 ? 2 : 3;
  mmd_pm1_flops(nx, ny, dim, true, *bf16_terms, passes, int8_flops, bf16_flops);
  return DVG_OK;
}

extern "C" size_t dvg_mmd_workspace_bytes(int64_t nx, int64_t ny, int dim) {
  if (nx <= 0 || ny <= 0 || dim <= 0 || dim % 32) return 0;
  return mmd_plan(nx, ny, dim).total;
}

extern "C" int dvg_mmd_fwd_bwd(const float* x, int64_t nx, const float* y, int64_t ny, int dim,
                               const dvg_mmd_cfg_t* cfg, float* loss_out, float* grad_x, void* ws, size_t ws_bytes,
                               dvg_stream_t stream) {
  DVG_REQUIRE(x && y && cfg && loss_out && ws, "mmd: null argument");
  DVG_REQUIRE(nx >= 2 && ny >= 2, "mmd: need at least 2 rows in x and y (nx=%lld ny=%lld)", (long long)nx, (long long)ny);
  DVG_REQUIRE(dim >= 32 && dim % 32 == 0 && dim <= 16384, "mmd: dim=%d must be a multiple of 32", dim);
  DVG_REQUIRE(cfg->n_kernels >= 1 && cfg->n_kernels <= 8, "mmd: n_kernels=%d not in [1,8]", cfg->n_kernels);
  const MmdPlan p = mmd_plan(nx, ny, dim);
  if (ws_bytes < p.total) { set_error("mmd: workspace %zu < %zu", ws_bytes, p.total); return DVG_E_WORKSPACE; }
  hipStream_t s = (hipStream_t)stream;
  char* w = (char*)ws;
  MmdArgs a;
  a.x = x; a.y = y; a.nx = nx; a.ny = ny; a.d = dim;
  a.sq = (float*)(w + p.off_sq);
  a.coef = (float*)(w + p.off_coef);
  a.n_kernels = cfg->n_kernels; a.squared = cfg->squared; a.reduce_mean = cfg->reduce_mean; a.biased = cfg->biased;
  a.pow2 = cfg->factor == 2.0f;
  a.loss_part = (double*)(w + p.off_loss);
  const int S_eff = p.w128 ? p.S2 : p.S;
  a.grad_part = grad_x ? (S_eff > 1 ? (float*)(w + p.off_grad) : grad_x) : nullptr;
  a.S = S_eff;
  a.dist_part = (double*)(w + p.off_dist);
  a.zi8 = (const int8_t*)(w + p.off_zi8);
  a.not_pm1 = (const int*)(w + p.off_flag);
  a.pm1_ok = p.pm1_ok;
  a.gate_main = 0;
  a.zt = (const uint16_t*)(w + p.off_zt);
  a.ztb_y = p.ztb_x;
  a.tab = (const uint4*)(w + p.off_tab);

  DVG_CHECK_HIP(hipMemsetAsync(w + p.off_flag, 0, sizeof(int), s));
  int loss_parts = (int)(p.S * (p.rbx + p.rby));
  if (p.w128) {
    if ((int)(p.S2 * p.z128 * (p.rb128x + p.rb128y)) > loss_parts) loss_parts = (int)(p.S2 * p.z128 * (p.rb128x + p.rb128y));
    if ((int)(p.S2 * (p.rbx + p.rby)) > loss_parts) loss_parts = (int)(p.S2 * (p.rbx + p.rby));
  }
  if (p.pm1_ok) {
    DVG_LAUNCH(K_MMD_PREP, mmd_prep_fused_kernel, dim3((unsigned)(p.ztb_x + p.ztb_y)), dim3(256), (size_t)32 * (dim + 16), s, a,
               (float*)(w + p.off_sq), (int8_t*)(w + p.off_zi8), (int*)(w + p.off_flag), (uint16_t*)(w + p.off_zt),
               p.w128 ? loss_parts : 0);
  } else {
    DVG_LAUNCH(K_MMD_PREP, mmd_prep_kernel, dim3((unsigned)ceil_div(nx + ny, 4)), dim3(256), 0, s, x, nx, y, ny, dim,
               (float*)(w + p.off_sq), (int8_t*)(w + p.off_zi8), (int*)(w + p.off_flag));
  }
  int ndist = 0;
  if (!(cfg->bandwidth > 0.f)) {
    ndist = (int)(p.S1 * p.GX1);
    const int pw = dim < MMD_I8_PANEL ? dim : MMD_I8_PANEL;
    const size_t lds_f = 2048 + sizeof(float) * (MMD_BJ + MMD_BI) * MMD_PITCH;
    const dim3 grid((unsigned)p.GX1, (unsigned)p.S1);
    if (p.pm1_ok) {
      const size_t lds_s = 2048 + ((size_t)(dim + 1) * 4 + 15) / 16 * 16 + (size_t)MMD_BJ * (pw + 16);
      const size_t lds_d = lds_f > lds_s ? lds_f : lds_s;
      auto launch = [&](auto kern) -> int {
        if (lds_d > 64 * 1024)
          DVG_CHECK_HIP(hipFuncSetAttribute((const void*)kern, hipFuncAttributeMaxDynamicSharedMemorySize, (int)lds_d));
        DVG_LAUNCH(K_MMD_DISTSUM, kern, grid, dim3(256), lds_d, s, a);
        return DVG_OK;
      };
      if (p.d256) {
        const size_t lds_2 = 2048 + ((size_t)(dim + 1) * 4 + 1023) / 1024 * 1024 + 2 * (size_t)32 * dim;
        const size_t lds_256 = lds_f > lds_2 ? lds_f : lds_2;
        auto launch256 = [&](auto kern) -> int {
          DVG_LAUNCH(K_MMD_DISTSUM, kern, grid, dim3(256), lds_256, s, a);
          return DVG_OK;
        };
        if (dim == 128) DVG_TRY(launch256(mmd_distsum_spin256_kernel<4>));
        else if (dim == 256) DVG_TRY(launch256(mmd_distsum_spin256_kernel<8>));
        else if (dim == 384) DVG_TRY(launch256(mmd_distsum_spin256_kernel<12>));
        else DVG_TRY(launch256(mmd_distsum_spin256_kernel<16>));
      } else
      if (dim <= 128) DVG_TRY(launch(mmd_distsum_spin_kernel<4>));
      else if (dim <= 512) DVG_TRY(launch(mmd_distsum_spin_kernel<16>));
      else DVG_TRY(launch(mmd_distsum_spin_kernel<32>));
    } else {
      const size_t lds_i = 2048 + (size_t)(MMD_BJ + MMD_BI) * (pw + 16);
      const size_t lds_d = lds_f > lds_i ? lds_f : lds_i;
      if (lds_d > 64 * 1024)
        DVG_CHECK_HIP(hipFuncSetAttribute((const void*)mmd_distsum_kernel, hipFuncAttributeMaxDynamicSharedMemorySize, (int)lds_d));
      DVG_LAUNCH(K_MMD_DISTSUM, mmd_distsum_kernel, grid, dim3(256), lds_d, s, a);
    }
  }
  DVG_LAUNCH(K_MMD_FINAL, mmd_bandwidth_table_kernel, dim3(1), dim3(256), 0, s, a, (const double*)(w + p.off_dist), ndist,
             (double)(nx + ny), cfg->bandwidth, cfg->factor, (float*)(w + p.off_coef),
             p.pm1_ok ? (uint4*)(w + p.off_tab) : (uint4*)nullptr);
  int rc;
  if (p.w128) {
    switch (dim / 128) {
      case 1: rc = launch_pair_w128<4, 4>(a, p, s); break;
      case 2: rc = launch_pair_w128<8, 8>(a, p, s); break;
      case 3: rc = launch_pair_w128<12, 12>(a, p, s); break;
      case 8: rc = p.z128 == 4 ? launch_pair_w128<32, 8, true>(a, p, s) : launch_pair_w128<32, 4>(a, p, s); break;
      default: rc = launch_pair_w128<16, 16>(a, p, s); break;
    }
    DVG_TRY(rc);
    MmdArgs g = a;
    g.gate_main = 1;
    MmdPlan pg = p;
    pg.S = p.S2;
    switch (p.nfb) {
      case 2: rc = launch_main<2>(g, pg, s); break;
      case 4: rc = launch_main<4>(g, pg, s); break;
      default: rc = launch_main<8>(g, pg, s); break;
    }
  } else if (p.pm1_ok) {
    const int fbt = dim / 32;
    if (dim % 128 == 0 && dim <= 512) {
      switch (dim / 128) {
        case 1: rc = launch_pair_fq<1>(a, p, s); break;
        case 2: rc = launch_pair_fq<2>(a, p, s); break;
        case 3: rc = launch_pair_fq<3>(a, p, s); break;
        default: rc = launch_pair_fq<4>(a, p, s); break;
      }
    } else if (fbt % 8 == 0) rc = launch_pair<8>(a, p, s);
    else if (fbt % 4 == 0) rc = launch_pair<4>(a, p, s);
    else if (fbt % 2 == 0) rc = launch_pair<2>(a, p, s);
    else rc = launch_pair<1>(a, p, s);
  } else {
    switch (p.nfb) {
      case 2: rc = launch_main<2>(a, p, s); break;
      case 4: rc = launch_main<4>(a, p, s); break;
      default: rc = launch_main<8>(a, p, s); break;
    }
  }
  DVG_TRY(rc);
  const int64_t numel = nx * (int64_t)dim;
  const unsigned fgrid = (grad_x && S_eff > 1) ? (unsigned)(ceil_div(numel, 256) > 2048 ? 2048 : ceil_div(numel, 256)) : 1u;
  DVG_LAUNCH(K_MMD_FINAL, mmd_final_kernel, dim3(fgrid), dim3(256), 0, s, (const double*)(w + p.off_loss),
             loss_parts, nx, ny, cfg->biased, loss_out, (const float*)(w + p.off_grad), S_eff, numel, grad_x);
  return DVG_OK;
}
```

### image-generation_amd/csrc/options.cpp

```cpp
#include <atomic>
#include <cstring>
#include <mutex>

#include "common.h"

namespace dvg {
namespace {
struct OptDef { const char* name; int64_t def; const char* doc; bool dev = false; };
const OptDef kDefs[OPT_COUNT] = {
    {"igemm_dma", 1, "float32 forward / data-gradient GEMM: 1 LDS-DMA staging (default), 0 register staging (tensors of 4 GiB and more always; A/B reference)", true},
    {"igemm_posmajor", 1, "position-major tiles (padding taps of small images never multiplied): 1 on, 0 pixel-major tiles"},
    {"igemm_thr128", 512, "blocks a launch must have for the 128x128 tile (the tests lower it to send small fixtures through that tile)", true},
    {"wgrad_dma", 1, "weight-gradient GEMMs: 1 LDS-DMA staging (default), 0 register staging (tensors of 4 GiB and more always)", true},
    {"dec_fold", 1, "decoder: Upsample(x2) + ConvTranspose as 4 class GEMMs with pre-summed taps (4/9 of the FLOPs)"},
    {"dec_d22", 1, "decoder: first ConvTranspose layer on 2x2 images as one dense map per image (16/36 of the FLOPs)"},
    {"dec_lc0", -1, "decoder: Linear composed with that map: -1 from 4096 rows up or rows x n_latents >= 2^20 (default), 0 never, 1 always"},
    {"mmd_w128", -1, "MMD: 128-row-block pair kernel: -1 by problem size (default), 0 never, 1 whenever the shape allows", true},
    {"mmd_d256", -1, "MMD: 256-row distance-sum kernel: -1 by problem size (default), 0 never, 1 whenever the shape allows", true},
    {"gibbs_generic", 0, "sampler: 1 forces the plain rolled reference schedule (no chains-side-by-side form for large graphs), 2 the lane-major schedule one row at a time instead of two passes of a class side by side, 3 the lane-major schedule whatever the size, 4 the chains-side-by-side schedule in 8-chain workgroups whatever the size (all bit-identical; A/B references)", true},
    {"side_stream", 1, "weight-gradient chains on the library's side stream (0 serialises everything on the caller's)"},
    {"enc_wino", -1, "encoder 3x3 layers in the Winograd F(2x2,3x3) form, forward, data gradient and weight gradient: -1 by size (default: evaluation-mode forward launches of 256 workgroups' worth of tiles or more, training launches of 512 or more), 0 never, 1 every launch the shape allows; forward / data gradient never in the bf16-input mode"},
    {"dec_wino", -1, "decoder Upsample(x2) + 3x3 layers in the Winograd form (9 of 16 transform positions), forward, data gradient and weight gradient: -1 from 8192 decoder rows up (default), 0 never, 1 whenever the shape allows"},
    {"enc_l0_fused", 1, "encoder layer 0: 1 = its output is recomputed by every pass that needs it (BatchNorm statistics, BN/pool/LeakyReLU, the backward sums, the weight gradient) and never stored (default), 0 = stored and re-read (rounds 1-2)", true},
    {"dec_tail_fused", 1, "decoder: 1 = the 8x8x32 stage's BatchNorm / Dropout / LeakyReLU (forward and backward) run inside the 32 -> 1 layer's kernels, its activated map and that map's gradient are never stored (default), 0 = separate passes (rounds 1-2)", true},
    {"wino_dynamic", 1, "Winograd forward / data-gradient launches deal their tile blocks dynamically (an atomic counter per grid row) instead of round-robin: a workgroup that gets its CU late takes fewer blocks (1 default, 0 = the static deal of rounds 3-4)", true},
    {"enc_wino4", 1, "every launch of the Winograd F(4x4,3x3) form -- forward, data gradient and weight gradient, encoder and decoder: 1 (default) the launches that run in the Winograd domain take it where the shape qualifies and their bit of the dev options enc_wino4_mask / dec_wino4_mask is set (36 position GEMMs per 4x4 output tile: 2.25 multiplies per output instead of 4.0; behind the decoder's upsample 25 of the 36), 0 none: the F(2x2,3x3) form everywhere"},
    {"enc_wino4_mask", 0x13c, "which encoder launches option enc_wino4 covers: bit l-1 the forward of layer l (1..3), bit 2+l its data gradient, bit 5+l its weight gradient (default 0x13c: layer 3's forward, every data gradient, layer 3's weight gradient -- the forwards of layers 1-2 gain nothing inside the step and their 7x float32 noise in front of two more max-pool stages moved the B = 1024 full-size gradient test from 4.6e-3 to 5.4e-3 of its 5e-3 bar; the weight gradients of layers 1-2 are level with the F(2x2,3x3) kernel)", true},
    {"enc_dgrad_cus", 0, "CUs the encoder's Winograd data-gradient launches are sized for (0: the measured constant of conv.h)", true},
    {"enc_wgrad_cus", 0, "CUs the encoder's Winograd weight-gradient launches are sized for (0: the measured constant of conv.h)", true},
    {"dec_wino4_mask", 0x2, "which of the decoder's Winograd launches behind the upsample take the F(4x4,3x3) form with 25 of 36 positions (option enc_wino4 != 0): bit 0 / 1 the forward of the 128 -> 64 / 64 -> 32 layer (bit 0 off: with it the full-size decoder's reconstruction is 2.97e-6 from float64, the bar is 2e-6), bit 2 / 3 their data gradients", true},
    {"wgrad_reduce_tiled", 1, "weight-gradient slab sums of at most 8 slabs and at least 256 tiles by the tiled one-thread-per-element kernels (same bits; 0: the 8-lanes-per-element kernels everywhere)", true},
    {"enc_bn_reduce_pooled", 1, "encoder BatchNorm/pool backward: the (sum dz, sum dz zhat) pass reads the pooled activations the forward kept (2 floats per element) instead of the four pre-BatchNorm outputs of every window (5); 0: the window form", true},
};
std::atomic<int64_t> g_val[OPT_COUNT];
std::once_flag g_once;
void init_once() {
  std::call_once(g_once, [] {
    for (int i = 0; i < OPT_COUNT; ++i) g_val[i].store(kDefs[i].def, std::memory_order_relaxed);
  });
}
}

int64_t opt(Opt id) {
  init_once();
  return g_val[id].load(std::memory_order_relaxed);
}
}

using namespace dvg;

namespace {
int nth(bool dev, int i) {
  for (int k = 0; k < OPT_COUNT; ++k)
    if (kDefs[k].dev == dev && i-- == 0) return k;
  return -1;
}
int count(bool dev) {
  int n = 0;
  for (int k = 0; k < OPT_COUNT; ++k) n += kDefs[k].dev == dev;
  return n;
}
int set_opt(bool dev, const char* what, const char* name, int64_t value) {
  DVG_REQUIRE(name, "%s: null name", what);
  init_once();
  for (int i = 0; i < OPT_COUNT; ++i)
    if (kDefs[i].dev == dev && !strcmp(name, kDefs[i].name)) { g_val[i].store(value, std::memory_order_relaxed); return DVG_OK; }
  set_error("%s: unknown option '%s'", what, name);
  return DVG_E_INVALID;
}
int get_opt(bool dev, const char* what, const char* name, int64_t* value) {
  DVG_REQUIRE(name && value, "%s: null argument", what);
  init_once();
  for (int i = 0; i < OPT_COUNT; ++i)
    if (kDefs[i].dev == dev && !strcmp(name, kDefs[i].name)) { *value = g_val[i].load(std::memory_order_relaxed); return DVG_OK; }
  set_error("%s: unknown option '%s'", what, name);
  return DVG_E_INVALID;
}
}

extern "C" int dvg_option_count(void) { return count(false); }
extern "C" const char* dvg_option_name(int index) { const int k = nth(false, index); return k >= 0 ? kDefs[k].name : nullptr; }
extern "C" const char* dvg_option_doc(int index) { const int k = nth(false, index); return k >= 0 ? kDefs[k].doc : nullptr; }
extern "C" int dvg_set_option(const char* name, int64_t value) { return set_opt(false, "dvg_set_option", name, value); }
extern "C" int dvg_get_option(const char* name, int64_t* value) { return get_opt(false, "dvg_get_option", name, value); }

extern "C" int dvg_dev_option_count(void) { return count(true); }
extern "C" const char* dvg_dev_option_name(int index) { const int k = nth(true, index); return k >= 0 ? kDefs[k].name : nullptr; }
extern "C" const char* dvg_dev_option_doc(int index) { const int k = nth(true, index); return k >= 0 ? kDefs[k].doc : nullptr; }
extern "C" int dvg_dev_set_option(const char* name, int64_t value) { return set_opt(true, "dvg_dev_set_option", name, value); }
extern "C" int dvg_dev_get_option(const char* name, int64_t* value) { return get_opt(true, "dvg_dev_get_option", name, value); }

extern "C" int dvg_reset_options(void) {
  init_once();
  for (int i = 0; i < OPT_COUNT; ++i) g_val[i].store(kDefs[i].def, std::memory_order_relaxed);
  return DVG_OK;
}
```

Before: 570,300.

## Compute MMD Gram of ±1 rows with FP4 scaled MFMA on packed e2m1 copies

```diff
diff --git a/image-generation_amd/csrc/common.h b/image-generation_amd/csrc/common.h
--- a/image-generation_amd/csrc/common.h
+++ b/image-generation_amd/csrc/common.h
@@ -86,7 +86,7 @@
 enum Opt : int {
   OPT_IGEMM_DMA = 0, OPT_IGEMM_POSMAJOR, OPT_IGEMM_THR128, OPT_WGRAD_DMA, OPT_DEC_FOLD, OPT_DEC_D22, OPT_DEC_LC0, OPT_MMD_W128,
   OPT_MMD_D256, OPT_GIBBS_GENERIC, OPT_SIDE_STREAM, OPT_ENC_WINO, OPT_DEC_WINO, OPT_ENC_L0_FUSED, OPT_DEC_TAIL_FUSED,
-  OPT_WINO_DYNAMIC, OPT_ENC_WINO4, OPT_ENC_WINO4_MASK, OPT_ENC_DGRAD_CUS, OPT_ENC_WGRAD_CUS, OPT_DEC_WINO4_MASK, OPT_WGRAD_REDUCE_TILED, OPT_ENC_BN_REDUCE_POOLED, OPT_COUNT
+  OPT_WINO_DYNAMIC, OPT_ENC_WINO4, OPT_ENC_WINO4_MASK, OPT_ENC_DGRAD_CUS, OPT_ENC_WGRAD_CUS, OPT_DEC_WINO4_MASK, OPT_WGRAD_REDUCE_TILED, OPT_ENC_BN_REDUCE_POOLED, OPT_MMD_GRAM_FP4, OPT_COUNT
 };
 int64_t opt(Opt id);
 
diff --git a/image-generation_amd/csrc/mmd.hip b/image-generation_amd/csrc/mmd.hip
--- a/image-generation_amd/csrc/mmd.hip
+++ b/image-generation_amd/csrc/mmd.hip
@@ -30,6 +30,7 @@
   const uint16_t* zt;
   int64_t ztb_y;
   const uint4* tab;
+  const uint8_t* zi4 = nullptr;
 };
 
 constexpr int MMD_BI = 32;
@@ -352,9 +353,17 @@
   if (threadIdx.x == 0) a.dist_part[(size_t)blockIdx.y * gridDim.x + blockIdx.x] = s;
 }
 
-template <int NST>
+typedef int i32x8 __attribute__((ext_vector_type(8)));
+__device__ __forceinline__ f32x16 mfma_fp4(const i32x4& za, const i32x4& zb, const f32x16& c) {
+  const i32x8 a8 = {za[0], za[1], za[2], za[3], 0, 0, 0, 0}, b8 = {zb[0], zb[1], zb[2], zb[3], 0, 0, 0, 0};
+  return __builtin_amdgcn_mfma_scale_f32_32x32x64_f8f6f4(a8, b8, c, 4, 4, 0, 127, 0, 127);
+}
+
+template <int NST, bool FP4 = false>
 __device__ __forceinline__ void mmd_distsum_spin256(const MmdArgs& a, unsigned char* dsm) {
-  constexpr int D = 32 * NST, CH = 32 * D, NPW = NST / 4;
+  static_assert(!FP4 || NST % 8 == 0, "FP4 rows: a wave's DMA piece is 1 KiB of a [32][d / 2] chunk");
+  constexpr int D = 32 * NST, P = FP4 ? D / 2 : D, NK = FP4 ? NST / 2 : NST, CH = 32 * P, NPW = CH / 4096;
+  using acc_t = std::conditional_t<FP4, f32x16, i32x16>;
   typedef __attribute__((address_space(3))) void lds_void;
   double* red = reinterpret_cast<double*>(dsm);
   float* Dtab = reinterpret_cast<float*>(dsm + 2048);
@@ -374,14 +383,15 @@
   }
   const int lane = threadIdx.x & 63, hh = lane >> 5, c = lane & 31;
   const int wave = __builtin_amdgcn_readfirstlane(threadIdx.x >> 6);
-  const __amdgpu_buffer_rsrc_t rsrc = __builtin_amdgcn_make_buffer_rsrc(const_cast<int8_t*>(a.zi8), 0, N * D, 0x00020000);
+  const unsigned char* zrows = FP4 ? reinterpret_cast<const unsigned char*>(a.zi4) : reinterpret_cast<const unsigned char*>(a.zi8);
+  const __amdgpu_buffer_rsrc_t rsrc = __builtin_amdgcn_make_buffer_rsrc(const_cast<unsigned char*>(zrows), 0, N * P, 0x00020000);
   int poff[NPW];
 #pragma unroll
   for (int q = 0; q < NPW; ++q) {
     const int byte = (wave * NPW + q) * 1024 + lane * 16;
-    const int r = byte / D, sl = (byte % D) >> 4;
-    const int f = (D % 256 == 0) ? (r & 15) : ((r >> 1) & 7);
-    poff[q] = r * D + ((sl ^ f) << 4);
+    const int r = byte / P, sl = (byte % P) >> 4;
+    const int f = (P % 256 == 0) ? (r & 15) : ((r >> 1) & 7);
+    poff[q] = r * P + ((sl ^ f) << 4);
   }
   auto issue = [&](int t, int buf) {
     unsigned char* dst = zbuf + buf * CH + wave * NPW * 1024;
@@ -389,7 +399,7 @@
     for (int q = 0; q < NPW; ++q)
       __builtin_amdgcn_raw_ptr_buffer_load_lds(rsrc, (lds_void*)(dst + q * 1024), 16, poff[q], t * CH, 0, 0);
   };
-  const int fc = (D % 256 == 0) ? (c & 15) : ((c >> 1) & 7);
+  const int fc = (P % 256 == 0) ? (c & 15) : ((c >> 1) & 7);
   constexpr int tb2 = 2048 + 2 * D;
   typedef __attribute__((address_space(3))) const float lds_cfloat;
   typedef __attribute__((address_space(3))) unsigned char lds_byte;
@@ -398,7 +408,7 @@
   uint32_t zaddr[8];
 #pragma unroll
   for (int j = 0; j < 8; ++j)
-    zaddr[j] = (uint32_t)(2048 + ((D + 1) * 4 + 1023) / 1024 * 1024) + (uint32_t)(c * D + ((((hh ^ fc) ^ (2 * j)) & 15) << 4));
+    zaddr[j] = (uint32_t)(2048 + ((D + 1) * 4 + 1023) / 1024 * 1024) + (uint32_t)(c * P + ((((hh ^ fc) ^ (2 * j)) & 15) << 4));
   double total = 0.0;
   __syncthreads();
   const int S = (int)gridDim.y, NB = (int)gridDim.x;
@@ -414,29 +424,30 @@
     const int k0 = lo > base ? lo - base : 0, k1 = hi - base < len ? hi - base : len;
     base += len;
     if (k1 <= k0) continue;
-    i32x4 xb[2][NST];
+    i32x4 xb[2][NK];
     bool vi[2];
 #pragma unroll
     for (int rs = 0; rs < 2; ++rs) {
       const int gi = g * 256 + wave * 64 + rs * 32 + c;
       vi[rs] = gi < N;
-      const int8_t* xrow = a.zi8 + (int64_t)(vi[rs] ? gi : N - 1) * D + hh * 16;
-#pragma unroll
-      for (int s = 0; s < NST; ++s) {
+      const unsigned char* xrow = zrows + (int64_t)(vi[rs] ? gi : N - 1) * P + hh * 16;
+#pragma unroll
+      for (int s = 0; s < NK; ++s) {
         const i32x4 w = *reinterpret_cast<const i32x4*>(xrow + s * 32);
 #pragma unroll
-        for (int u = 0; u < 4; ++u) xb[rs][s][u] = (int)((((uint32_t)w[u] << 1) & 0xFEFEFEFEu) ^ 0xFCFCFCFCu);
+        for (int u = 0; u < 4; ++u)
+          xb[rs][s][u] = FP4 ? (int)((uint32_t)w[u] ^ 0xEEEEEEEEu) : (int)((((uint32_t)w[u] << 1) & 0xFEFEFEFEu) ^ 0xFCFCFCFCu);
       }
     }
     const int t0 = g * 8 + by + S * k0, t_end = g * 8 + by + S * k1, t_own_end = g * 8 + 8;
     float part[2] = {0.f, 0.f};
     double segsum[2] = {0.0, 0.0};
-    auto lookups = [&](const i32x16& g0, const i32x16& g1, int t, bool masked) {
+    auto lookups = [&](const acc_t& g0, const acc_t& g1, int t, bool masked) {
       float p0 = 0.f, p1 = 0.f;
 #pragma unroll
       for (int r = 0; r < 16; ++r) {
-        const float d0 = *reinterpret_cast<lds_cfloat*>((uintptr_t)(uint32_t)(g0[r] + tb2));
-        const float d1 = *reinterpret_cast<lds_cfloat*>((uintptr_t)(uint32_t)(g1[r] + tb2));
+        const float d0 = *reinterpret_cast<lds_cfloat*>((uintptr_t)(uint32_t)((int)g0[r] + tb2));
+        const float d1 = *reinterpret_cast<lds_cfloat*>((uintptr_t)(uint32_t)((int)g1[r] + tb2));
         const bool vj = !masked || t * 32 + crow(r, hh) < N;
         p0 += vj ? d0 : 0.f;
         p1 += vj ? d1 : 0.f;
@@ -448,7 +459,8 @@
     issue(t0, 0);
     int tp = -1, since_flush = 0;
     constexpr int PF = NST >= 16 ? 4 : (NST >= 8 ? 2 : 1);
-    auto chunk = [&](int t, auto bufc, const i32x16 (&prev)[2], i32x16 (&cur)[2]) {
+    static_assert(PF < NK, "operand prefetch distance");
+    auto chunk = [&](int t, auto bufc, const acc_t (&prev)[2], acc_t (&cur)[2]) {
       constexpr int buf = decltype(bufc)::value;
       asm volatile("s_waitcnt vmcnt(0)" ::: "memory");
       __syncthreads();
@@ -456,23 +468,28 @@
       auto zread = [&](int st) -> i32x4 {
         return *reinterpret_cast<lds_ci32x4*>((uintptr_t)(zaddr[st & 7] + (uint32_t)(buf * CH + (st >> 3) * 256)));
       };
-      auto rb = [](int st) { return (16 * st) / NST; };
-      i32x4 zr[NST];
+      auto rb = [](int st) { return (16 * st) / NK; };
+      i32x4 zr[NK];
       float lk0[16], lk1[16], p0 = 0.f, p1 = 0.f;
 #pragma unroll
       for (int s = 0; s < PF; ++s) zr[s] = zread(s);
       __builtin_amdgcn_sched_barrier(0);
 #pragma unroll
-      for (int s = 0; s < NST; ++s) {
+      for (int s = 0; s < NK; ++s) {
 #pragma unroll
         for (int r = rb(s); r < rb(s + 1); ++r) {
-          lk0[r] = *reinterpret_cast<lds_cfloat*>((uintptr_t)(uint32_t)(prev[0][r] + tb2));
-          lk1[r] = *reinterpret_cast<lds_cfloat*>((uintptr_t)(uint32_t)(prev[1][r] + tb2));
-        }
-        if (s + PF < NST) zr[s + PF] = zread(s + PF);
+          lk0[r] = *reinterpret_cast<lds_cfloat*>((uintptr_t)(uint32_t)((int)prev[0][r] + tb2));
+          lk1[r] = *reinterpret_cast<lds_cfloat*>((uintptr_t)(uint32_t)((int)prev[1][r] + tb2));
+        }
+        if (s + PF < NK) zr[s + PF] = zread(s + PF);
         __builtin_amdgcn_sched_barrier(0);
-        cur[0] = __builtin_amdgcn_mfma_i32_32x32x32_i8(zr[s], xb[0][s], s == 0 ? (i32x16){0} : cur[0], 0, 0, 0);
-        cur[1] = __builtin_amdgcn_mfma_i32_32x32x32_i8(zr[s], xb[1][s], s == 0 ? (i32x16){0} : cur[1], 0, 0, 0);
+        if constexpr (FP4) {
+          cur[0] = mfma_fp4(zr[s], xb[0][s], s == 0 ? (f32x16){0} : cur[0]);
+          cur[1] = mfma_fp4(zr[s], xb[1][s], s == 0 ? (f32x16){0} : cur[1]);
+        } else {
+          cur[0] = __builtin_amdgcn_mfma_i32_32x32x32_i8(zr[s], xb[0][s], s == 0 ? (i32x16){0} : cur[0], 0, 0, 0);
+          cur[1] = __builtin_amdgcn_mfma_i32_32x32x32_i8(zr[s], xb[1][s], s == 0 ? (i32x16){0} : cur[1], 0, 0, 0);
+        }
         if (s >= PF) {
 #pragma unroll
           for (int r = rb(s - PF); r < rb(s - PF + 1); ++r) { p0 += lk0[r]; p1 += lk1[r]; }
@@ -480,7 +497,7 @@
         __builtin_amdgcn_sched_barrier(0);
       }
 #pragma unroll
-      for (int r = rb(NST - PF); r < 16; ++r) { p0 += lk0[r]; p1 += lk1[r]; }
+      for (int r = rb(NK - PF); r < 16; ++r) { p0 += lk0[r]; p1 += lk1[r]; }
       const float wgt = tp < 0 ? 0.0f : (tp < t_own_end ? 1.0f : 2.0f);
       part[0] = fmaf(p0, wgt, part[0]);
       part[1] = fmaf(p1, wgt, part[1]);
@@ -491,8 +508,8 @@
         since_flush = 0;
       }
     };
-    i32x16 accp[2], accq[2];
-    accp[0] = (i32x16){0}; accp[1] = (i32x16){0};
+    acc_t accp[2], accq[2];
+    accp[0] = (acc_t){0}; accp[1] = (acc_t){0};
     bool last_in_q = false;
     for (int t = t0; t < t_end; t += 2 * S) {
       chunk(t, std::integral_constant<int, 0>{}, accp, accq);
@@ -511,10 +528,10 @@
   if (threadIdx.x == 0) a.dist_part[(size_t)by * gridDim.x + bx] = sum;
 }
 
-template <int NST>
+template <int NST, bool FP4 = false>
 __global__ __launch_bounds__(256, 2) void mmd_distsum_spin256_kernel(MmdArgs a) {
   extern __shared__ __align__(16) unsigned char dsm[];
-  if (*a.not_pm1 == 0) mmd_distsum_spin256<NST>(a, dsm);
+  if (*a.not_pm1 == 0) mmd_distsum_spin256<NST, FP4>(a, dsm);
   else mmd_distsum_generic(a, dsm, false);
 }
 
@@ -720,7 +737,7 @@
 
 __global__ __launch_bounds__(256) void mmd_prep_fused_kernel(MmdArgs a, float* __restrict__ sq, int8_t* __restrict__ zi8,
                                                              int* __restrict__ not_pm1, uint16_t* __restrict__ zt,
-                                                             int zero_loss_parts) {
+                                                             int zero_loss_parts, uint8_t* __restrict__ zi4) {
   extern __shared__ __align__(16) unsigned char prep_smem[];
   const int tid = threadIdx.x, lane = tid & 63, wave = tid >> 6, d = a.d, pitch = d + 16;
   for (int64_t e = (int64_t)blockIdx.x * 256 + tid; e < 3 * (int64_t)zero_loss_parts; e += (int64_t)gridDim.x * 256)
@@ -750,6 +767,9 @@
                          (w.w > 0.f ? 0x01000000u : 0xff000000u);
       *reinterpret_cast<uint32_t*>(prep_smem + (wave + 4 * u) * pitch + 4 * k) = z;
       if (row < cnt) reinterpret_cast<uint32_t*>(zi8 + (goff + row) * d)[k] = z;
+      if (zi4 && row < cnt)
+        reinterpret_cast<uint16_t*>(zi4 + (goff + row) * (d >> 1))[k] =
+            (uint16_t)(0x2222u | ((z >> 4) & 0x8u) | ((z >> 8) & 0x80u) | ((z >> 12) & 0x800u) | ((z >> 16) & 0x8000u));
     }
   }
   if (__any(bad) && lane == 0) atomicOr(not_pm1, 1);
@@ -1133,13 +1153,14 @@
   }
 }
 
-template <int NST, int NFT, bool ONE = false>
+template <int NST, int NFT, bool ONE = false, bool FP4 = false>
 struct W128 {
   static constexpr int D = 32 * NST;
+  static constexpr int P = FP4 ? D / 2 : D;
   static constexpr int TABN = D + 3;
   static constexpr int TAB_BYTES = ((ONE ? 1 : 2) * TABN * 8 + 1023) / 1024 * 1024;
   static constexpr int RED_BYTES = 2048;
-  static constexpr int Z8_BYTES = 32 * D;
+  static constexpr int Z8_BYTES = 32 * P;
   static constexpr int ZT_BYTES = 64 * 32 * NFT;
   static constexpr int NSTG = 3;
   static constexpr int OFF_RED = TAB_BYTES, OFF_Z8 = OFF_RED + RED_BYTES, OFF_ZT = OFF_Z8 + NSTG * Z8_BYTES;
@@ -1152,10 +1173,11 @@
                                    (void __attribute__((address_space(3)))*)lds_wave_base, 16, 0, 0);
 }
 
-template <int NST, int NFT, bool ONE = false>
+template <int NST, int NFT, bool ONE = false, bool FP4 = false>
 __device__ __forceinline__ void mmd_pm1_w128_body(const MmdArgs& a, unsigned char* smem) {
-  using L = W128<NST, NFT, ONE>;
-  constexpr int D = L::D;
+  using L = W128<NST, NFT, ONE, FP4>;
+  static_assert(!FP4 || (NST == NFT && NST % 8 == 0), "FP4 Gram: one k-step per two feature tiles, 1 KiB DMA pieces");
+  constexpr int D = L::D, P = L::P, NK = FP4 ? NST / 2 : NST;
   typedef __attribute__((address_space(3))) void lds_void;
   typedef __attribute__((address_space(3))) unsigned char lds_byte;
   typedef int i32x2 __attribute__((ext_vector_type(2)));
@@ -1214,27 +1236,33 @@
     const uint32_t lo = rn_bf16(w - __uint_as_float(hi));
     reinterpret_cast<uint2*>(smem)[e] = make_uint2(v.x, hi | (lo >> 16));
   }
-  i32x4 xb[NST];
+  const unsigned char* zrows = FP4 ? reinterpret_cast<const unsigned char*>(a.zi4) : reinterpret_cast<const unsigned char*>(a.zi8);
+  i32x4 xb[NK];
   {
-    const int8_t* xrow = a.zi8 + (goff_i + (vi ? gi : cnt_i - 1)) * D + hh * 16;
-#pragma unroll
-    for (int s = 0; s < NST; ++s) xb[s] = *reinterpret_cast<const i32x4*>(xrow + s * 32);
-  }
-
-  constexpr int NZ8 = NST / 4, NZT = NFT / 2;
+    const unsigned char* xrow = zrows + (goff_i + (vi ? gi : cnt_i - 1)) * P + hh * 16;
+#pragma unroll
+    for (int s = 0; s < NK; ++s) {
+      xb[s] = *reinterpret_cast<const i32x4*>(xrow + s * 32);
+      if constexpr (FP4) xb[s] ^= (i32x4){(int)0xEEEEEEEE, (int)0xEEEEEEEE, (int)0xEEEEEEEE, (int)0xEEEEEEEE};
+    }
+  }
+  int sc_a = 127, sc_b = 127;
+  asm volatile("" : "+v"(sc_a), "+v"(sc_b));
+
+  constexpr int NZ8 = L::Z8_BYTES / 4096, NZT = NFT / 2;
   int z8off[NZ8], ztoff0;
 #pragma unroll
   for (int q = 0; q < NZ8; ++q) {
     const int byte = (wave * NZ8 + q) * 1024 + lane * 16;
-    const int r = byte / D, sl = (byte % D) >> 4;
-    const int fz = (D % 256 == 0) ? (r & 15) : ((r >> 1) & 7);
-    z8off[q] = r * D + ((sl ^ fz) << 4);
+    const int r = byte / P, sl = (byte % P) >> 4;
+    const int fz = (P % 256 == 0) ? (r & 15) : ((r >> 1) & 7);
+    z8off[q] = r * P + ((sl ^ fz) << 4);
   }
   {
     const int f = wave * NZT * 16 + (lane >> 2), sl = lane & 3;
     ztoff0 = f * 64 + ((sl ^ ((f >> 2) & 3)) << 4);
   }
-  const __amdgpu_buffer_rsrc_t rsrc8 = __builtin_amdgcn_make_buffer_rsrc(const_cast<int8_t*>(a.zi8), 0, (int)((a.nx + a.ny) * D), 0x00020000);
+  const __amdgpu_buffer_rsrc_t rsrc8 = __builtin_amdgcn_make_buffer_rsrc(const_cast<unsigned char*>(zrows), 0, (int)((a.nx + a.ny) * P), 0x00020000);
   const __amdgpu_buffer_rsrc_t rsrct = __builtin_amdgcn_make_buffer_rsrc(
       const_cast<uint16_t*>(a.zt), 0, (int)((a.ztb_y + (a.ny + 127) / 128 * 4) * (int64_t)D * 64), 0x00020000);
   const uint32_t lds0 = (uint32_t)__builtin_amdgcn_readfirstlane((int)(uint32_t)(uintptr_t)(lds_byte*)smem);
@@ -1242,7 +1270,7 @@
   auto z8_soff = [&](int t) -> int {
     t = t < tl_i ? t : tl_i;
     const bool cx = t < ncx_i;
-    return ((cx ? 0 : nx_i) + (cx ? t : t - ncx_i) * 32) * D;
+    return ((cx ? 0 : nx_i) + (cx ? t : t - ncx_i) * 32) * P;
   };
   auto zt_soff = [&](int t) -> int {
     t = t < tl_i ? t : tl_i;
@@ -1264,24 +1292,35 @@
       __builtin_amdgcn_raw_ptr_buffer_load_lds(rsrct, (lds_void*)(uintptr_t)(dst + q * 1024), 16, ztoff0, so + q * 1024, 0, 0);
   };
 
-  const int fz_c = (D % 256 == 0) ? (c & 15) : ((c >> 1) & 7);
+  const int fz_c = (P % 256 == 0) ? (c & 15) : ((c >> 1) & 7);
   const int sw_c = (c >> 2) & 3;
   const int aoff0 = c * 64 + ((hh ^ sw_c) << 4), aoff1 = c * 64 + (((2 + hh) ^ sw_c) << 4);
-  constexpr int ZSW = (D % 256 == 0) ? 16 : 8;
-  constexpr int NZB = ZSW / 2 < NST ? ZSW / 2 : NST;
+  constexpr int ZSW = (P % 256 == 0) ? 16 : 8;
+  constexpr int NZB = ZSW / 2 < NK ? ZSW / 2 : NK;
   int zlow[NZB];
 #pragma unroll
-  for (int m = 0; m < NZB; ++m) zlow[m] = c * D + (((2 * m + hh) ^ fz_c) << 4);
+  for (int m = 0; m < NZB; ++m) zlow[m] = c * P + (((2 * m + hh) ^ fz_c) << 4);
 
   auto gram = [&](int stg) -> i32x16 {
     const unsigned char* z = z8buf + stg * L::Z8_BYTES;
-    i32x16 acc = {0};
-#pragma unroll
-    for (int s = 0; s < NST; ++s) {
-      const i32x4 za = *reinterpret_cast<const i32x4*>(z + zlow[s % NZB] + (s / NZB) * (ZSW * 16));
-      acc = __builtin_amdgcn_mfma_i32_32x32x32_i8(za, xb[s], acc, 0, 0, 0);
-    }
-    return acc;
+    if constexpr (FP4) {
+      f32x16 acc = {0};
+#pragma unroll
+      for (int s = 0; s < NK; ++s) {
+        const i32x4 za = *reinterpret_cast<const i32x4*>(z + zlow[s % NZB] + (s / NZB) * (ZSW * 16));
+        const i32x8 a8 = {za[0], za[1], za[2], za[3], 0, 0, 0, 0}, b8 = {xb[s][0], xb[s][1], xb[s][2], xb[s][3], 0, 0, 0, 0};
+        acc = __builtin_amdgcn_mfma_scale_f32_32x32x64_f8f6f4(a8, b8, acc, 4, 4, 0, 127, 0, 127);
+      }
+      return __builtin_bit_cast(i32x16, acc);
+    } else {
+      i32x16 acc = {0};
+#pragma unroll
+      for (int s = 0; s < NK; ++s) {
+        const i32x4 za = *reinterpret_cast<const i32x4*>(z + zlow[s % NZB] + (s / NZB) * (ZSW * 16));
+        acc = __builtin_amdgcn_mfma_i32_32x32x32_i8(za, xb[s], acc, 0, 0, 0);
+      }
+      return acc;
+    }
   };
 
   f32x16 G[NFT];
@@ -1309,8 +1348,8 @@
     for (int r = 0; r < 16; ++r) {
       const int jl = crow(r, hho);
       int v = S[r];
-      v = jl == dloc ? -(D + 4) : v;
-      v = jl < m.nj ? v : -(D + 2);
+      v = jl == dloc ? (FP4 ? __float_as_int((float)(2 * (D + 4))) : -(D + 4)) : v;
+      v = jl < m.nj ? v : (FP4 ? __float_as_int((float)(2 * (D + 2))) : -(D + 2));
       S[r] = v;
     }
   };
@@ -1319,7 +1358,7 @@
   uint32_t hm_prev = 0;
   constexpr int NTERM = 2;
   auto look_issue = [&](const i32x16& S, int r, const unsigned char* tb) -> i32x2 {
-    return *reinterpret_cast<const i32x2*>(tb + __mul24(S[r], -4));
+    return *reinterpret_cast<const i32x2*>(tb + (FP4 ? 2 * (int)__int_as_float(S[r]) : __mul24(S[r], -4)));
   };
   auto look_use = [&](const i32x2& e, int r, i32x4 (&Bn)[2][NTERM]) {
     lsum += __int_as_float(e[0]);
@@ -1376,6 +1415,8 @@
     auto rb = [](int ft) { return ft >= NFT - 1 ? 16 : (16 * ft + NFT - 2) / (NFT - 1); };
     constexpr int RMAX = (16 + NFT - 2) / (NFT - 1);
     constexpr int GPT = NST / NFT;
+    auto gram_tile = [](int ft) { return !FP4 || (ft & 1) == 0; };
+    auto gram_step = [](int ft) { return FP4 ? ft / 2 : ft * GPT; };
     struct Carry {
       int z8so, ztso;
       uint32_t z8dst, ztdst;
@@ -1441,7 +1482,8 @@
 #pragma unroll
       for (int ft = 0; ft < NFT; ++ft) {
 #pragma unroll
-        for (int u = 0; u < GPT; ++u) asm volatile("" ::"v"(zc[u]));
+        for (int u = 0; u < GPT; ++u)
+          if (gram_tile(ft)) asm volatile("" ::"v"(zc[u]));
         asm volatile("" ::"v"(ac[0]), "v"(ac[1]));
         if (ft > 0) {
 #pragma unroll
@@ -1454,6 +1496,13 @@
           if constexpr (GPT > 1) {
             if (ft == 0 && u == 0) Snext = (i32x16){0};
             Snext = __builtin_amdgcn_mfma_i32_32x32x32_i8(zc[u], xb[ft * GPT + u], Snext, 0, 0, 0);
+          } else if constexpr (FP4) {
+            if (ft == 0)
+              asm volatile("v_mfma_scale_f32_32x32x64_f8f6f4 %0, %1, %2, 0, %3, %4 op_sel_hi:[0,0,0] cbsz:4 blgp:4"
+                           : "=&v"(Snext) : "v"(zc[u]), "v"(xb[ft / 2]), "v"(sc_a), "v"(sc_b));
+            else if (gram_tile(ft))
+              asm volatile("v_mfma_scale_f32_32x32x64_f8f6f4 %0, %1, %2, %0, %3, %4 op_sel_hi:[0,0,0] cbsz:4 blgp:4"
+                           : "+v"(Snext) : "v"(zc[u]), "v"(xb[ft / 2]), "v"(sc_a), "v"(sc_b));
           } else
           if (ft == 0 && u == 0)
             asm volatile("v_mfma_i32_32x32x32_i8 %0, %1, %2, 0" : "=&v"(Snext) : "v"(zc[u]), "v"(xb[ft * GPT + u]));
@@ -1465,7 +1514,8 @@
           an[0] = *reinterpret_cast<const i32x4*>(ad.a0 + (ft + 1) * 2048);
           an[1] = *reinterpret_cast<const i32x4*>(ad.a1 + (ft + 1) * 2048);
 #pragma unroll
-          for (int u = 0; u < GPT; ++u) zn[u] = zread(ad, (ft + 1) * GPT + u);
+          for (int u = 0; u < GPT; ++u)
+            if (gram_tile(ft + 1)) zn[u] = zread(ad, gram_step(ft + 1) + u);
         } else {
           if constexpr (GPT > 1) {
             asm volatile("s_waitcnt vmcnt(%0)" ::"n"(NZ8 + NZT) : "memory");
@@ -1517,7 +1567,8 @@
         for (int u = 0; u < RMAX; ++u) ent[u] = enew[u];
         ac[0] = an[0]; ac[1] = an[1];
 #pragma unroll
-        for (int u = 0; u < GPT; ++u) zc[u] = zn[u];
+        for (int u = 0; u < GPT; ++u)
+          if (gram_tile(ft + 1 < NFT ? ft + 1 : 0)) zc[u] = zn[u];
         __builtin_amdgcn_sched_group_barrier(0x100, 2, 0);
         __builtin_amdgcn_sched_group_barrier(0x020, 2, 0);
 #pragma unroll
@@ -1594,11 +1645,11 @@
   }
 }
 
-template <int NST, int NFT, bool ONE = false>
+template <int NST, int NFT, bool ONE = false, bool FP4 = false>
 __global__ __launch_bounds__(256, 1) void mmd_pair_w128_kernel(MmdArgs a) {
   extern __shared__ __align__(16) unsigned char w128_smem[];
   if (*a.not_pm1 != 0) return;
-  mmd_pm1_w128_body<NST, NFT, ONE>(a, w128_smem);
+  mmd_pm1_w128_body<NST, NFT, ONE, FP4>(a, w128_smem);
 }
 
 template <int NFB>
@@ -1657,6 +1708,8 @@
 struct MmdPlan {
   int nfb, zslices, S, S1;
   bool d256;
+  bool fp4;
+  size_t off_zi4;
   int64_t rbx, rby, GX1;
   size_t off_sq, off_coef, off_dist, off_loss, off_grad, off_flag, off_zi8, off_zt, off_tab, total;
   int pm1_ok;
@@ -1722,6 +1775,8 @@
     const int64_t t256 = ceil_div(nx + ny, 256);
     p.d256 = p.pm1_ok && env != 0 && d % 128 == 0 && d <= 512 && (t256 >= 32 || env == 1) && (nx + ny) * (int64_t)d < 2147483647LL;
   }
+  const bool fp4_shape = p.pm1_ok && (d == 256 || d == 512);
+  p.fp4 = fp4_shape && (p.d256 || p.w128) && opt(OPT_MMD_GRAM_FP4) != 0;
   if (p.d256) {
     p.GX1 = 64;
     S1 = 8;
@@ -1758,6 +1813,7 @@
   p.off_zi8 = o; o = align_up(o + (size_t)(nx + ny) * (size_t)d, 256);
   p.off_zt = o; o = align_up(o + (p.pm1_ok ? (size_t)(p.ztb_x + p.ztb_y) * (size_t)d * 32 * sizeof(uint16_t) : 0), 256);
   p.off_tab = o; o = align_up(o + (p.pm1_ok ? 2 * (size_t)(d + 1) * sizeof(uint4) : 0), 256);
+  p.off_zi4 = o; o = align_up(o + (fp4_shape ? (size_t)(nx + ny) * (size_t)(d / 2) : 0), 256);
   p.total = o;
   return p;
 }
@@ -1812,10 +1868,10 @@
   return DVG_OK;
 }
 
-template <int NST, int NFT, bool ONE = false>
+template <int NST, int NFT, bool ONE = false, bool FP4 = false>
 static int launch_pair_w128(const MmdArgs& a, const MmdPlan& p, hipStream_t s) {
-  auto kern = mmd_pair_w128_kernel<NST, NFT, ONE>;
-  constexpr int lds = W128<NST, NFT, ONE>::LDS_BYTES;
+  auto kern = mmd_pair_w128_kernel<NST, NFT, ONE, FP4>;
+  constexpr int lds = W128<NST, NFT, ONE, FP4>::LDS_BYTES;
   if (lds > 64 * 1024)
     DVG_CHECK_HIP(hipFuncSetAttribute((const void*)kern, hipFuncAttributeMaxDynamicSharedMemorySize, lds));
   DVG_LAUNCH_WORK(K_MMD_PM1, mmd_pm1_work(a, 2, NST / NFT), kern, dim3((unsigned)(p.rb128x + p.rb128y), (unsigned)p.S2, NST / NFT),
@@ -1890,6 +1946,7 @@
   a.zt = (const uint16_t*)(w + p.off_zt);
   a.ztb_y = p.ztb_x;
   a.tab = (const uint4*)(w + p.off_tab);
+  a.zi4 = p.fp4 ? (const uint8_t*)(w + p.off_zi4) : nullptr;
 
   DVG_CHECK_HIP(hipMemsetAsync(w + p.off_flag, 0, sizeof(int), s));
   int loss_parts = (int)(p.S * (p.rbx + p.rby));
@@ -1900,7 +1957,7 @@
   if (p.pm1_ok) {
     DVG_LAUNCH(K_MMD_PREP, mmd_prep_fused_kernel, dim3((unsigned)(p.ztb_x + p.ztb_y)), dim3(256), (size_t)32 * (dim + 16), s, a,
                (float*)(w + p.off_sq), (int8_t*)(w + p.off_zi8), (int*)(w + p.off_flag), (uint16_t*)(w + p.off_zt),
-               p.w128 ? loss_parts : 0);
+               p.w128 ? loss_parts : 0, p.fp4 ? (uint8_t*)(w + p.off_zi4) : (uint8_t*)nullptr);
   } else {
     DVG_LAUNCH(K_MMD_PREP, mmd_prep_kernel, dim3((unsigned)ceil_div(nx + ny, 4)), dim3(256), 0, s, x, nx, y, ny, dim,
                (float*)(w + p.off_sq), (int8_t*)(w + p.off_zi8), (int*)(w + p.off_flag));
@@ -1927,7 +1984,8 @@
           DVG_LAUNCH(K_MMD_DISTSUM, kern, grid, dim3(256), lds_256, s, a);
           return DVG_OK;
         };
-        if (dim == 128) DVG_TRY(launch256(mmd_distsum_spin256_kernel<4>));
+        if (p.fp4) DVG_TRY(dim == 256 ? launch256(mmd_distsum_spin256_kernel<8, true>) : launch256(mmd_distsum_spin256_kernel<16, true>));
+        else if (dim == 128) DVG_TRY(launch256(mmd_distsum_spin256_kernel<4>));
         else if (dim == 256) DVG_TRY(launch256(mmd_distsum_spin256_kernel<8>));
         else if (dim == 384) DVG_TRY(launch256(mmd_distsum_spin256_kernel<12>));
         else DVG_TRY(launch256(mmd_distsum_spin256_kernel<16>));
@@ -1950,10 +2008,10 @@
   if (p.w128) {
     switch (dim / 128) {
       case 1: rc = launch_pair_w128<4, 4>(a, p, s); break;
-      case 2: rc = launch_pair_w128<8, 8>(a, p, s); break;
+      case 2: rc = p.fp4 ? launch_pair_w128<8, 8, false, true>(a, p, s) : launch_pair_w128<8, 8>(a, p, s); break;
       case 3: rc = launch_pair_w128<12, 12>(a, p, s); break;
       case 8: rc = p.z128 == 4 ? launch_pair_w128<32, 8, true>(a, p, s) : launch_pair_w128<32, 4>(a, p, s); break;
-      default: rc = launch_pair_w128<16, 16>(a, p, s); break;
+      default: rc = p.fp4 ? launch_pair_w128<16, 16, false, true>(a, p, s) : launch_pair_w128<16, 16>(a, p, s); break;
     }
     DVG_TRY(rc);
     MmdArgs g = a;
diff --git a/image-generation_amd/csrc/options.cpp b/image-generation_amd/csrc/options.cpp
--- a/image-generation_amd/csrc/options.cpp
+++ b/image-generation_amd/csrc/options.cpp
@@ -31,6 +31,7 @@
     {"dec_wino4_mask", 0x2, "which of the decoder's Winograd launches behind the upsample take the F(4x4,3x3) form with 25 of 36 positions (option enc_wino4 != 0): bit 0 / 1 the forward of the 128 -> 64 / 64 -> 32 layer (bit 0 off: with it the full-size decoder's reconstruction is 2.97e-6 from float64, the bar is 2e-6), bit 2 / 3 their data gradients", true},
     {"wgrad_reduce_tiled", 1, "weight-gradient slab sums of at most 8 slabs and at least 256 tiles by the tiled one-thread-per-element kernels (same bits; 0: the 8-lanes-per-element kernels everywhere)", true},
     {"enc_bn_reduce_pooled", 1, "encoder BatchNorm/pool backward: the (sum dz, sum dz zhat) pass reads the pooled activations the forward kept (2 floats per element) instead of the four pre-BatchNorm outputs of every window (5); 0: the window form", true},
+    {"mmd_gram_fp4", 1, "MMD: exact Gram of +-1 rows on the FP4 matrix pipe (scaled 32x32x64 MFMA on a packed e2m1 copy of the rows: the same integers at half the operand bytes and k-steps) in the 256-row distance-sum kernel and the 128-row-block pair kernel at d = 256, 512 (default); 0: the int8 form (A/B reference, same bits)", true},
 };
 std::atomic<int64_t> g_val[OPT_COUNT];
 std::once_flag g_once;
```

New measurement: 591,700, median of 6. 1.04x the previous value.
